# CycloneBoy/pdf_table

Measured on AMD Instinct MI355X. Metric: pages/s, higher is better.
Workload: dtype bf16

## Files before the change

include/pdftable_hip.h:

```cpp
#ifndef PDFTABLE_HIP_H
#define PDFTABLE_HIP_H

#include <stddef.h>
#include <stdint.h>

#ifdef __cplusplus
extern "C" {
#endif

#define PT_OK 0
#define PT_ERR_INVALID 1
#define PT_ERR_HIP 2
#define PT_ERR_STATE 3
#define PT_ERR_FORMAT 4

typedef struct pt_engine pt_engine;
typedef void* pt_stream;

int pt_engine_create(int device_id, pt_engine** out);
void pt_engine_destroy(pt_engine* e);
const char* pt_last_error(void);
int pt_abi_version(void);
int pt_engine_check(pt_engine* e);
int pt_engine_set_lstm_cluster(pt_engine* e, int on);
// ... 100 lines not shown
int pt_rec_forward_net(pt_engine* e, const uint16_t* d_gray, int n, int32_t* d_ids, float* d_maxlogit, pt_stream stream);
int pt_rec_preprocess(pt_engine* e, const uint8_t* d_pages_rgb, int n_pages, int h, int w, const pt_rec_line* d_lines,
                      const int64_t* h_crop_px, int n_lines, uint16_t* d_gray, pt_stream stream);

#define PT_CVIT_W 804
#define PT_CVIT_CHUNK_W 300
#define PT_CVIT_CHUNK_STEP 252
#define PT_CVIT_T 201
#define PT_CVIT_NCLS 7644
int pt_rec_cvit_forward(pt_engine* e, const uint8_t* d_pages_rgb, int n_pages, int h, int w, const pt_rec_line* d_lines,
                        const int64_t* h_crop_px, const int32_t* h_crop_wh, int n_lines, int32_t* d_ids, float* d_maxlogit,
                        pt_stream stream);
int pt_rec_cvit_forward_crops(pt_engine* e, const uint8_t* d_crops_rgb, const pt_rec_line* d_lines, const int64_t* h_crop_px,
                              const int32_t* h_crop_wh, int n_lines, int32_t* d_ids, float* d_maxlogit, pt_stream stream);
int pt_rec_cvit_forward_net(pt_engine* e, const float* d_gray, int layout, int n_lines, const int32_t* h_text_w, int32_t* d_ids,
                            float* d_maxlogit, pt_stream stream);
int pt_rec_cvit_preprocess_crops(pt_engine* e, const uint8_t* d_crops_rgb, const pt_rec_line* d_lines, const int64_t* h_crop_px,
                                 int n_lines, float* d_gray, pt_stream stream);

typedef struct pt_rec_pp_item {
  int32_t line;
  int32_t resized_w;
  int32_t img_w;
  int32_t reserved;
  int64_t out_off;
} pt_rec_pp_item;
int pt_rec_pp_preprocess(pt_engine* e, const uint8_t* d_pages_rgb, int n_pages, int h, int w, const pt_rec_line* d_lines,
                         const int64_t* h_crop_px, int n_lines, const pt_rec_pp_item* d_items, int n_items, int img_h,
                         int max_img_w, float* d_out, pt_stream stream);
int pt_rec_pp_preprocess_crops(pt_engine* e, const uint8_t* d_crops_rgb, const pt_rec_line* d_lines, const int64_t* h_crop_px,
                               int n_lines, const pt_rec_pp_item* d_items, int n_items, int img_h, int max_img_w, float* d_out,
                               pt_stream stream);

typedef struct pt_tsr_table {
  double minv[6];
  int32_t page, x0, y0, crop_w, crop_h, reserved;
} pt_tsr_table;

int pt_tsr_preprocess(pt_engine* e, const uint8_t* d_pages_rgb, int n_pages, int ph, int pw, const pt_tsr_table* d_tables,
                      int n, int inp_h, int inp_w, int bgr, uint16_t* d_out_bf16, pt_stream stream);

#define PT_TSR_CS_SMALL 8
#define PT_TSR_CS_FEAT 256
int pt_tsr_forward_net(pt_engine* e, const uint16_t* d_input_bf16, int n, int H, int W, float* d_hm, float* d_st,
                       float* d_wh, float* d_ax, float* d_cr, float* d_reg, pt_stream stream);

int pt_tsr_forward_net_wireless(pt_engine* e, const uint16_t* d_input_bf16, int n, int H, int W, float* d_hm, float* d_st,
                                float* d_wh, float* d_ax, float* d_cr, float* d_reg, pt_stream stream);

#define PT_TSR_MAX_CELLS 3000
int pt_tsr_decode(pt_engine* e, const float* d_hm, const float* d_st, const float* d_wh, const float* d_ax,
                  const float* d_cr, const float* d_reg, int n, int h, int w, int wiz_rev, float vis_thresh,
                  int32_t* d_counts, float* d_dets, float* d_logi, pt_stream stream);

int pt_tsr_forward_decode(pt_engine* e, const uint16_t* d_input_bf16, int n, int in_h, int in_w, int wiz_rev,
                          float vis_thresh, int32_t* d_counts, float* d_dets, float* d_logi, pt_stream stream);

int pt_centernet_forward_net(pt_engine* e, const uint16_t* d_input_bf16, int n, int H, int W, float* d_hm, float* d_v2c, float* d_c2v,
                             float* d_reg, pt_stream stream);

#define PT_CENTERNET_MAX_CELLS 1000
int pt_centernet_decode(pt_engine* e, const float* d_hm, const float* d_v2c, const float* d_c2v, const float* d_reg, int n, int h, int w,
                        const double* d_affine, int32_t* d_counts, float* d_cells, pt_stream stream);

int pt_tsr_process(pt_engine* e, const float* d_logi, const float* d_dets, const int32_t* h_counts, int n_tables,
                   int use_2dpe, float* d_logic, float* d_stacked, pt_stream stream);

int pt_op_conv2d(pt_engine* e, const uint16_t* d_in, int B, int H, int W, int Cin, const uint16_t* d_w_tiled,
                 const float* d_bias, int N, int ks, int stride, uint16_t* d_out, int out_cstride, int out_coff,
                 int rep, int shuffle_cout, const uint16_t* d_res, int res_mode, int relu, int split, int out_lo_off,
                 pt_stream stream);
int pt_op_conv1x1_ex(pt_engine* e, const uint16_t* d_in, int B, int H, int W, int Cin, const uint16_t* d_w_tiled, const float* d_bias,
                     int N, uint16_t* d_out, float* d_out_f32, int out_cstride, int n_valid, const float* d_res_f32, int relu,
                     const int32_t* d_ylimit, pt_stream stream);

int pt_op_dcn(pt_engine* e, const uint16_t* d_in, const float* d_om, int B, int H, int W, int C, const uint16_t* d_w_tiled,
              const float* d_bias, int N, uint16_t* d_out, int relu, int split, pt_stream stream);

int pt_op_dwconvt_up_add(pt_engine* e, const uint16_t* d_in, const float* d_w, const uint16_t* d_add, uint16_t* d_out, int B, int h, int w, int C,
                         int f, int split, pt_stream stream);
int pt_op_dcn_up_add(pt_engine* e, const uint16_t* d_in, const float* d_om, int B, int H, int W, int C, const uint16_t* d_w_tiled,
                     const float* d_bias, int N, uint16_t* d_out, int relu, int split, const uint16_t* d_up_in, int up_h, int up_w,
                     const float* d_up_w, int up_f, pt_stream stream);

int pt_op_stem7x7(pt_engine* e, const uint16_t* d_in, int B, int H, int W, const uint16_t* d_w, const float* d_bias,
                  uint16_t* d_out, int split, pt_stream stream);
int pt_op_maxpool3x3s2(pt_engine* e, const uint16_t* d_in, int B, int H, int W, int C, uint16_t* d_out, int split,
                       pt_stream stream);
int pt_op_db_head_final(pt_engine* e, const uint16_t* d_in, int B, int H, int W, const void* d_w, const float* d_bias,
                        float* d_prob, float* d_logits, int split, pt_stream stream);

int pt_op_dwconv(pt_engine* e, const uint16_t* d_in, int B, int H, int W, int C, const float* d_w_taps, const float* d_bias, int k,
                 int stride, int act, uint16_t* d_out, int split, pt_stream stream);
int pt_op_add(pt_engine* e, const uint16_t* d_a, const uint16_t* d_b, uint16_t* d_out, long long npix, int C, int split, pt_stream stream);
int pt_op_maxpool(pt_engine* e, const uint16_t* d_in, int B, int H, int W, int C, int k, int stride, int pad, uint16_t* d_out,
                  int split, pt_stream stream);
int pt_op_avgpool(pt_engine* e, const uint16_t* d_in, int B, int H, int W, int C, int k, uint16_t* d_out, int split, pt_stream stream);
int pt_op_chan_mean(pt_engine* e, const uint16_t* d_in, int B, int HW, int C, float* d_scratch, uint16_t* d_mean, int split, pt_stream stream);
int pt_op_chan_mean_scratch_floats(int B, int C);
int pt_op_scale_channels(pt_engine* e, const uint16_t* d_in, const uint16_t* d_gate, int B, int HW, int C, uint16_t* d_out,
                         int split, pt_stream stream);
int pt_op_act(pt_engine* e, const uint16_t* d_in, long long n_elems, int kind, float alpha, float beta, uint16_t* d_out, int C, int split,
              pt_stream stream);
int pt_op_copy_channels(pt_engine* e, const uint16_t* d_src, long long npix, int src_cstride, int src_coff, uint16_t* d_dst, int dst_cstride, int dst_coff,
                        int n, pt_stream stream);
int pt_op_upsample_nearest(pt_engine* e, const uint16_t* d_in, int B, int H, int W, int C, int factor, uint16_t* d_out, pt_stream stream);
int pt_op_mul(pt_engine* e, const uint16_t* d_a, const uint16_t* d_b, uint16_t* d_out, long long n_elems, int C, int split, pt_stream stream);
int pt_copy_bytes(pt_engine* e, const void* src, void* dst, long long nbytes, pt_stream stream);
int pt_op_layernorm(pt_engine* e, const uint16_t* d_in, long long rows, int c_pad, int c, const float* d_gamma, const float* d_beta, float eps,
                    uint16_t* d_out, int split, pt_stream stream);
int pt_op_softmax(pt_engine* e, const uint16_t* d_in, long long rows, int c_pad, int c, float* d_out_f32, uint16_t* d_out_bf16, int split, pt_stream stream);
int pt_op_attention(pt_engine* e, const uint16_t* d_qkv, int B, int T, int heads, int d, int qkv_cstride, float scale, uint16_t* d_out, int out_cstride,
                    int split, pt_stream stream);

int pt_op_cvit_mlp(pt_engine* e, const uint16_t* d_xb, long long rows, int C, const uint16_t* d_w1, const float* d_b1, const uint16_t* d_w2p,
                   const float* d_b2, float* d_x, pt_stream stream);
int pt_op_cvit_attention(pt_engine* e, const uint16_t* d_qkv, int nchunks, uint16_t* d_out, int split, pt_stream stream);
int pt_op_cvit_dwconv_ln(pt_engine* e, const float* d_x, int B, int H, int W, int C, const float* d_w49, const float* d_bias, const float* d_g,
                         const float* d_beta, uint16_t* d_out, int split, pt_stream stream);
int pt_op_cvit_ln(pt_engine* e, const float* d_x, long long rows, int C, const float* d_g, const float* d_beta, float eps, uint16_t* d_out, int split,
                  int mode, int H, int W, const int32_t* d_cmap, pt_stream stream);

int pt_op_lstm(pt_engine* e, const uint16_t* d_pregates, int pg_cstride, const uint16_t* d_r_packed, int T, int B, int H, int dirs, int reverse,
               uint16_t* d_y, int y_cstride, int split, pt_stream stream);
int pt_op_lstm_packed_elems(int H, int dirs, int split);

int pt_op_conv2d_rect(pt_engine* e, const uint16_t* d_in, int B, int H, int W, int Cin, const uint16_t* d_w_tiled, const float* d_bias, int N, int kh,
                      int kw, int sh, int sw, uint16_t* d_out, int out_cstride, int out_coff, int act, int split, int out_lo_off, pt_stream stream);
int pt_op_dwconv_rect(pt_engine* e, const uint16_t* d_in, int B, int H, int W, int C, const float* d_w_taps, const float* d_bias, int k, int sh, int sw,
                      int act, uint16_t* d_out, int split, pt_stream stream);
int pt_op_pool_rect(pt_engine* e, const uint16_t* d_in, int B, int H, int W, int C, int kind, int kh, int kw, uint16_t* d_out, int split,
                    pt_stream stream);

int pt_op_conv2d_large(pt_engine* e, const uint16_t* d_in, int B, int H, int W, int Cin, const uint16_t* d_w_tiled, const float* d_bias, int N, int kh,
                       int kw, uint16_t* d_out, int out_cstride, int out_coff, int act, int split, int out_lo_off, pt_stream stream);

int pt_op_affine_act(pt_engine* e, const uint16_t* d_in, long long npix, int Cpad, int C, const float* d_s1, const float* d_b1, const float* d_s2,
                     const float* d_b2, int act, uint16_t* d_out, int split, pt_stream stream);
int pt_op_db_tail(pt_engine* e, const uint16_t* d_in, int B, int H, int W, int Cpad, int C, int C1, const float* d_w1, const float* d_b1,
                  const float* d_w2, const float* d_b2, float* d_out, int split, pt_stream stream);

#define PT_CLS_SLOTS 4
#define PT_CLS_MAX_CLASSES 16
typedef struct pt_cls_image {
  int64_t offset;
  int32_t h, w;
} pt_cls_image;

int pt_cls_preprocess(pt_engine* e, const uint8_t* d_base, const pt_cls_image* d_images, int n, int max_h, int max_w,
                      int out_h, int out_w, uint16_t* d_out_bf16, pt_stream stream);
int pt_cls_forward_net(pt_engine* e, int slot, const uint16_t* d_input_bf16, int n, int in_h, int in_w, int textline,
                       float* d_logits, int* n_classes, pt_stream stream);
int pt_cls_forward(pt_engine* e, int slot, const uint8_t* d_base, const pt_cls_image* d_images, int n, int max_h, int max_w,
                   int out_h, int out_w, int textline, float* d_logits, int* n_classes, pt_stream stream);
int pt_cls_forward_lines(pt_engine* e, int slot, const uint8_t* d_pages_rgb, int n_pages, int h, int w,
                         const pt_rec_line* d_lines, const int64_t* h_crop_px, int n_lines, int max_crop_h, int max_crop_w,
                         int out_h, int out_w, int textline, float* d_logits, int* n_classes, pt_stream stream);
int pt_cls_forward_lines_direct(pt_engine* e, int slot, const uint8_t* d_pages_rgb, int n_pages, int h, int w,
                                const pt_rec_line* d_lines, int n_lines, int max_crop_h, int max_crop_w, int out_h, int out_w,
                                int textline, float* d_logits, int* n_classes, pt_stream stream);

#define PT_PROF_CONV3X3 0
#define PT_PROF_CONV1X1 1
#define PT_PROF_STEM 2
#define PT_PROF_OTHER 3
#define PT_PROF_NCLASS 4
// ... 33 lines not shown
```

pdf_table_amd/csrc/c_api.hip:

```cpp
#include <stdarg.h>
#include <stdio.h>
#include <stdlib.h>

#include <cmath>

#include "common.h"

namespace PT_FMT_NS {
namespace api {

static int ensure(void** buf, size_t* cap, size_t need);

int pt_engine_check(pt_engine* e) {
  PT_REQUIRE(e, "pt_engine_check: null engine");
  if (e->lstm_err && *e->lstm_err) {
    *e->lstm_err = 0;
    e->lstm_cluster = 0;
    pt_set_error("lstm_cluster_kernel: a workgroup waited > 2^22 polls for its peers -- the launch was not co-resident "
                 "(GPU shared with another process or stream?).  The recognition results since the last check are invalid; "
                 "this engine now uses the streaming LSTM kernel (pt_engine_set_lstm_cluster(e, 0)): run the batch again");
    return PT_ERR_HIP;
  }
  return PT_OK;
}
// ... 894 lines not shown
  bf16_t* xin = reinterpret_cast<bf16_t*>(e->cls_direct_in);
  for (int i0 = 0; i0 < n_lines; i0 += mb) {
    const int nb = (n_lines - i0) < mb ? (n_lines - i0) : mb;
    {
      PtProfScope ps(e, s, PT_PROF_OTHER, 0, "cls line resize+norm");
      rc = pt_launch_cls_line_resize_norm(d_pages_rgb, h, w, d_lines + i0, nb, max_crop_h, max_crop_w, out_h, out_w, e->cls_lut, x3, xin, s);
      if (rc != PT_OK) return rc;
    }
    rc = pt_pplcnet_forward_net(e, slot, xin, nb, out_h, out_w, textline, d_logits + (size_t)i0 * PT_CLS_MAX_CLASSES, n_classes, s,
                                PT_ARENA_CLS);
    if (rc != PT_OK) return rc;
  }
  return PT_OK;
}

int pt_op_conv2d(pt_engine* e, const uint16_t* d_in, int B, int H, int W, int Cin, const uint16_t* d_w_tiled,
                 const float* d_bias, int N, int ks, int stride, uint16_t* d_out, int out_cstride, int out_coff,
                 int rep, int shuffle_cout, const uint16_t* d_res, int res_mode, int relu, int split, int out_lo_off,
                 pt_stream stream) {
  PT_REQUIRE(e != nullptr, "pt_op_conv2d: null engine");
  ConvDesc d;
  d.in = d_in; d.B = B; d.H = H; d.W = W; d.Cin = Cin; d.w = d_w_tiled; d.bias = d_bias; d.N = N; d.ks = ks;
  d.stride = stride; d.out = d_out; d.out_cstride = out_cstride; d.out_coff = out_coff; d.rep = rep;
  d.shuffle_cout = shuffle_cout; d.res = d_res; d.res_mode = res_mode; d.relu = relu;
  d.split = split; d.out_lo_off = out_lo_off;
  return pt_launch_conv(e, d, reinterpret_cast<hipStream_t>(stream));
}

int pt_op_conv1x1_ex(pt_engine* e, const uint16_t* d_in, int B, int H, int W, int Cin, const uint16_t* d_w_tiled, const float* d_bias,
                     int N, uint16_t* d_out, float* d_out_f32, int out_cstride, int n_valid, const float* d_res_f32, int relu,
                     const int32_t* d_ylimit, pt_stream stream) {
  PT_REQUIRE(e != nullptr, "pt_op_conv1x1_ex: null engine");
  ConvDesc d;
  d.in = d_in; d.B = B; d.H = H; d.W = W; d.Cin = Cin; d.w = d_w_tiled; d.bias = d_bias; d.N = N; d.ks = 1; d.stride = 1;
  d.out = d_out_f32 ? nullptr : d_out; d.out_f32 = d_out_f32; d.out_cstride = out_cstride; d.n_valid = n_valid; d.res_f32 = d_res_f32;
  d.relu = relu; d.ylimit = d_ylimit;
  return pt_launch_conv(e, d, reinterpret_cast<hipStream_t>(stream));
}

int pt_op_stem7x7(pt_engine* e, const uint16_t* d_in, int B, int H, int W, const uint16_t* d_w, const float* d_bias,
                  uint16_t* d_out, int split, pt_stream stream) {
  PT_REQUIRE(e != nullptr, "pt_op_stem7x7: null engine");
  return pt_launch_stem7x7(e, d_in, B, H, W, d_w, d_bias, d_out, split, reinterpret_cast<hipStream_t>(stream));
}

int pt_op_maxpool3x3s2(pt_engine* e, const uint16_t* d_in, int B, int H, int W, int C, uint16_t* d_out, int split,
                       pt_stream stream) {
  PT_REQUIRE(e && d_in && d_out, "pt_op_maxpool3x3s2: bad arguments");
  return pt_launch_maxpool3x3s2(d_in, B, H, W, C, d_out, split, reinterpret_cast<hipStream_t>(stream));
}

int pt_op_db_head_final(pt_engine* e, const uint16_t* d_in, int B, int H, int W, const void* d_w, const float* d_bias,
                        float* d_prob, float* d_logits, int split, pt_stream stream) {
  PT_REQUIRE(e && d_in && d_w && d_bias && (d_prob || d_logits), "pt_op_db_head_final: bad arguments");
  return pt_launch_db_head_final(d_in, B, H, W, d_w, d_bias, d_prob, d_logits, split, reinterpret_cast<hipStream_t>(stream));
}

int pt_op_dcn(pt_engine* e, const uint16_t* d_in, const float* d_om, int B, int H, int W, int C, const uint16_t* d_w_tiled,
              const float* d_bias, int N, uint16_t* d_out, int relu, int split, pt_stream stream) {
  PT_REQUIRE(e && d_in && d_om && d_w_tiled && d_bias && d_out, "pt_op_dcn: null argument");
  PT_REQUIRE(B > 0 && H > 0 && W > 0, "pt_op_dcn: empty map (B=%d H=%d W=%d)", B, H, W);
  return pt_launch_dcn_fused(e, d_in, d_om, d_w_tiled, d_bias, d_out, B, H, W, C, N, split, relu, reinterpret_cast<hipStream_t>(stream));
}

int pt_op_dwconvt_up_add(pt_engine* e, const uint16_t* d_in, const float* d_w, const uint16_t* d_add, uint16_t* d_out, int B, int h, int w, int C,
                         int f, int split, pt_stream stream) {
  PT_REQUIRE(e && d_in && d_w && d_out, "pt_op_dwconvt_up_add: null argument");
  PT_REQUIRE(B > 0 && h > 0 && w > 0 && C > 0, "pt_op_dwconvt_up_add: empty map (B=%d h=%d w=%d C=%d)", B, h, w, C);
  return pt_launch_dwconvt_up_add(d_in, d_w, d_add, d_out, B, h, w, C, f, split, reinterpret_cast<hipStream_t>(stream));
}

int pt_op_dcn_up_add(pt_engine* e, const uint16_t* d_in, const float* d_om, int B, int H, int W, int C, const uint16_t* d_w_tiled,
                     const float* d_bias, int N, uint16_t* d_out, int relu, int split, const uint16_t* d_up_in, int up_h, int up_w,
                     const float* d_up_w, int up_f, pt_stream stream) {
  PT_REQUIRE(e && d_in && d_om && d_w_tiled && d_bias && d_out && d_up_in && d_up_w, "pt_op_dcn_up_add: null argument");
  PT_REQUIRE(B > 0 && H > 0 && W > 0, "pt_op_dcn_up_add: empty map (B=%d H=%d W=%d)", B, H, W);
  PT_REQUIRE(split == 0, "pt_op_dcn_up_add: the (hi | lo) modes keep the two launches (pt_op_dcn, pt_op_dwconvt_up_add)");
  PT_REQUIRE((up_f == 2 || up_f == 4) && up_h > 0 && up_w > 0 && up_h * up_f == H && up_w * up_f == W,
             "pt_op_dcn_up_add: a %dx%d map times %d is not the %dx%d output", up_h, up_w, up_f, H, W);
  return pt_launch_dcn_fused(e, d_in, d_om, d_w_tiled, d_bias, d_out, B, H, W, C, N, split, relu, reinterpret_cast<hipStream_t>(stream), nullptr, nullptr,
                             d_up_in, d_up_w, up_f);
}

int pt_profile_enable(pt_engine* e, int on) {
  PT_REQUIRE(e != nullptr, "pt_profile_enable: null engine");
  PT_REQUIRE(on >= 0 && on < 2 + PT_PROF_NCLASS, "pt_profile_enable: mode %d out of range", on);
  if (on && !e->prof.h_lims)
    PT_HIP_CHECK(hipHostMalloc(reinterpret_cast<void**>(&e->prof.h_lims), PtProfile::MAX_LIMS * sizeof(int), hipHostMallocDefault));
  e->prof.on = on;
  return PT_OK;
}

int pt_profile_read_labels(pt_engine* e, char* buf, int cap) {
  PT_REQUIRE(e && buf && cap > 0, "pt_profile_read_labels: bad arguments");
  PT_HIP_CHECK(hipDeviceSynchronize());
  struct Row { double ms = 0, flop = 0, bytes = 0; long long n = 0; };
  std::map<std::string, Row> rows;
  for (auto& p : e->prof.pending) {
    float ms = 0.f;
    if (hipEventElapsedTime(&ms, p.a, p.b) != hipSuccess) continue;
    double fl = p.flop;
    if (p.lim_slot >= 0 && p.rows > 0) {
      const int lim = e->prof.h_lims[p.lim_slot];
      fl *= (double)(lim < 0 ? 0 : (lim > p.rows ? p.rows : lim)) / p.rows;
    }
    Row& r = rows[p.label];
    r.ms += ms; r.flop += fl; r.bytes += p.bytes; r.n += 1;
  }
  std::string text;
  char line[160];
  for (auto& kv : rows) {
    snprintf(line, sizeof(line), "%s\t%lld\t%.6f\t%.6e\t%.6e\n", kv.first.c_str(), kv.second.n, kv.second.ms, kv.second.flop, kv.second.bytes);
    text += line;
  }
  PT_REQUIRE((int)text.size() + 1 <= cap, "pt_profile_read_labels: %d bytes needed, %d given", (int)text.size() + 1, cap);
  memcpy(buf, text.c_str(), text.size() + 1);
  for (auto& p : e->prof.pending) {
    (void)hipEventDestroy(p.a);
    (void)hipEventDestroy(p.b);
  }
  e->prof.pending.clear();
  e->prof.n_lims = 0;
  for (int i = 0; i < PT_PROF_NCLASS; ++i) { e->prof.ms[i] = 0; e->prof.launches[i] = 0; e->prof.flop[i] = 0; }
  return PT_OK;
}

int pt_profile_read(pt_engine* e, double* ms_per_class, long long* launches_per_class, double* flop_per_class) {
  PT_REQUIRE(e != nullptr, "pt_profile_read: null engine");
  PT_HIP_CHECK(hipDeviceSynchronize());
  const bool verbose = getenv("PT_PROF_VERBOSE") != nullptr;
  std::map<std::string, std::pair<double, int>> by_label;
  for (auto& p : e->prof.pending) {
    float ms = 0.f;
    if (hipEventElapsedTime(&ms, p.a, p.b) == hipSuccess) {
      if (verbose) { auto& r = by_label[p.label]; r.first += ms; r.second += 1; }
      e->prof.ms[p.cls] += ms;
      e->prof.launches[p.cls] += 1;
      double fl = p.flop;
      if (p.lim_slot >= 0 && p.rows > 0) {
        const int lim = e->prof.h_lims[p.lim_slot];
        fl *= (double)(lim < 0 ? 0 : (lim > p.rows ? p.rows : lim)) / p.rows;
      }
      e->prof.flop[p.cls] += fl;
    }
    (void)hipEventDestroy(p.a);
    (void)hipEventDestroy(p.b);
  }
  e->prof.pending.clear();
  e->prof.n_lims = 0;
  if (verbose)
    for (auto& kv : by_label)
      fprintf(stderr, "[pt_prof] %-40s n=%5d total=%9.3f ms avg=%8.4f ms\n", kv.first.c_str(), kv.second.second, kv.second.first,
              kv.second.first / kv.second.second);
  for (int i = 0; i < PT_PROF_NCLASS; ++i) {
    if (ms_per_class) ms_per_class[i] = e->prof.ms[i];
    if (launches_per_class) launches_per_class[i] = e->prof.launches[i];
    if (flop_per_class) flop_per_class[i] = e->prof.flop[i];
    e->prof.ms[i] = 0;
    e->prof.launches[i] = 0;
    e->prof.flop[i] = 0;
  }
  return PT_OK;
}

}
}
// ... 1 lines not shown
```

pdf_table_amd/csrc/common.h:

```cpp
#pragma once
#include <hip/hip_runtime.h>
#include <stdint.h>
#include <string.h>

#include <map>
#include <string>
#include <vector>

#include "../../include/pdftable_hip.h"
#include "act16.h"

typedef uint16_t bf16_t;

void pt_set_error(const char* fmt, ...);

#define PT_HIP_CHECK(expr)                                                                  \
  do {                                                                                      \
    hipError_t _e = (expr);                                                                 \
    if (_e != hipSuccess) {                                                                 \
      pt_set_error("%s failed: %s (%s:%d)", #expr, hipGetErrorString(_e), __FILE__, __LINE__); \
      return PT_ERR_HIP;                                                                    \
    }                                                                                       \
  } while (0)

// ... 138 lines not shown
  int lstm_max_cl = 0;
  int dcn_mfma = 0;
  int mtl_kv_fp8 = 0;
  int lstm_cluster = 1;
  void* rec_zero[2] = {nullptr, nullptr};
  bool rec_zero_valid[2] = {false, false};
  hipEvent_t rec_zero_ready[2] = {nullptr, nullptr};
  void* rec_limits = nullptr; size_t rec_limits_cap = 0;
  int rec_ragged = 1;
  std::vector<int> cvit_maps[16][2];
  int cvit_slot = 0;
  PtPinnedRing stage_ring;
  void* mtl_state = nullptr;
};

namespace PT_FMT_NS {

__device__ __forceinline__ void pt_warp_sample(const uint8_t* __restrict__ src, int ph, int pw, const double* m, int x, int y, int v[3]) {
  const double X0 = m[0] * x + m[1] * y + m[2];
  const double Y0 = m[3] * x + m[4] * y + m[5];
  double W = m[6] * x + m[7] * y + m[8];
  W = W != 0. ? 32. / W : 0.;
  const double fX = fmax(-2147483648., fmin(2147483647., X0 * W));
  const double fY = fmax(-2147483648., fmin(2147483647., Y0 * W));
  const long long Xi = (long long)rint(fX), Yi = (long long)rint(fY);
  const long long sx = Xi >> 5, sy = Yi >> 5;
  const int ax = (int)(Xi & 31), ay = (int)(Yi & 31);
  const int w00 = (32 - ay) * (32 - ax) * 32, w01 = (32 - ay) * ax * 32, w10 = ay * (32 - ax) * 32, w11 = ay * ax * 32;
  int acc[3] = {0, 0, 0};
  auto tap = [&](long long yy, long long xx, int wgt) {
    if (wgt && yy >= 0 && yy < ph && xx >= 0 && xx < pw) {
      const uint8_t* p = src + ((size_t)yy * pw + xx) * 3;
      acc[0] += p[0] * wgt; acc[1] += p[1] * wgt; acc[2] += p[2] * wgt;
    }
  };
  tap(sy, sx, w00); tap(sy, sx + 1, w01); tap(sy + 1, sx, w10); tap(sy + 1, sx + 1, w11);
#pragma unroll
  for (int c = 0; c < 3; ++c) {
    const int t = (acc[c] + (1 << 14)) >> 15;
    v[c] = t < 0 ? 0 : (t > 255 ? 255 : t);
  }
}

struct ConvDesc {
  const bf16_t* in = nullptr;
  int B = 0, H = 0, W = 0, Cin = 0;
  const bf16_t* in_more[3] = {nullptr, nullptr, nullptr};
  int seg_c[4] = {0, 0, 0, 0};
  int nseg = 1;
  const bf16_t* w = nullptr;
  const float* bias = nullptr;
  int N = 0;
  int ks = 3;
  int stride = 1;
  bf16_t* out = nullptr;
  int out_cstride = 0;
  int out_coff = 0;
  int rep = 1;
  int shuffle_cout = 0;
  const bf16_t* res = nullptr;
  int res_mode = 0;
  int relu = 0;
  const float* slope = nullptr;
  int pool = 0;
  const int* ylimit = nullptr;
  const int* xlimit = nullptr;
  const int* xlimit_cols = nullptr;
  const int* xlimit_rows = nullptr;
  const int* block_list = nullptr;
  int split = 0;
  int out_lo_off = 0;
  const void* head_w = nullptr;
  const float* head_b = nullptr;
  float* head_prob = nullptr;
  float* head_logits = nullptr;
  float* argmax_part = nullptr;
  int n_valid = 0;
  float* out_f32 = nullptr;
  const float* res_f32 = nullptr;
  unsigned tap_mask[8] = {0, 0, 0, 0, 0, 0, 0, 0};
  int xp_store = 0;
  int alg_n = 0;
  double alg_scale = 1.0;
};
int pt_launch_conv(pt_engine* e, const ConvDesc& d, hipStream_t s);
int pt_launch_crnn_conv01(pt_engine* e, const bf16_t* gray, int n, const float* w64x9, const float* b0, const bf16_t* w1, const float* b1, bf16_t* p1,
                          const int* xlimit, const int* xlimit_cols, hipStream_t s);
int pt_launch_dwpw(pt_engine* e, const bf16_t* in, int B, int H, int W, int C, const float* dw_w, const float* dw_b, int k, int stride, int dw_act,
                   const ConvDesc& pw, hipStream_t s);

int pt_launch_stem7x7(pt_engine* e, const bf16_t* in, int B, int H, int W, const bf16_t* w, const float* bias,
                      bf16_t* out, int split, hipStream_t s, int stride = 2, int n_valid = 0);

int pt_launch_det_preprocess(const uint8_t* pages, int n, int h, int w, int nh, int nw, int flavour, int split,
                             bf16_t* out, hipStream_t s);
int pt_launch_dcn_fused(pt_engine* e, const bf16_t* x, const float* om, const bf16_t* w, const float* bias, bf16_t* out,
                        int B, int H, int W, int C, int N, int split, int relu, hipStream_t s, const bf16_t* omw = nullptr, const float* omb = nullptr,
                        const bf16_t* up_in = nullptr, const float* up_w = nullptr, int up_f = 0);
bool pt_dcn_fuses_om(const pt_engine* e, int C, int split);
bool pt_dcn_fuses_up(const pt_engine* e, int C, int N, int split);
int pt_launch_dwconvt_up_add(const bf16_t* in, const float* w, const bf16_t* add, bf16_t* out, int B, int h, int wd, int C, int f, int split,
                             hipStream_t s);
int pt_launch_maxpool3x3s2(const bf16_t* in, int B, int H, int W, int C, bf16_t* out, int split, hipStream_t s);
int pt_launch_stem7x7_pool(pt_engine* e, const bf16_t* in, int B, int H, int W, const bf16_t* w, const float* bias, bf16_t* out,
                           hipStream_t s);
int pt_launch_db_head_final(const bf16_t* in, int B, int H, int W, const void* w4x64, const float* bias, float* prob,
                            float* logits, int split, hipStream_t s);
int pt_launch_db_head_mfma(const bf16_t* in, int B, int H, int W, const bf16_t* w3, const float* b3, const bf16_t* w6,
                           const float* b6, float* prob, float* logits, hipStream_t s, uint32_t* bitmap = nullptr, float thresh = 0.f);
int pt_launch_bitmap(const float* prob, int n, int H, int W, float thresh, int dilate, uint32_t* bitmap,
                     hipStream_t s);
int pt_launch_box_scores(const float* prob, int n, int H, int W, const float* boxes, int nb, float* scores,
                         hipStream_t s);

#define PT_SE_CHUNKS 64
int pt_launch_stem3x3s2(const bf16_t* in, const float* w, const float* b, bf16_t* out, int B, int H, int W, int split,
                        hipStream_t s, int variant);
int pt_launch_dwconv(const bf16_t* in, const float* w, const float* b, bf16_t* out, int B, int H, int W, int C, int k,
                     int stride, int act, int split, hipStream_t s, const float* slope);
int pt_launch_se(const bf16_t* x, const float* w1, const float* b1, const float* w2, const float* b2, float* gate,
                 bf16_t* out, int B, int HW, int C, int split, hipStream_t s, int hidden, int mode, float* part);
int pt_launch_add(const bf16_t* a, const bf16_t* b, bf16_t* out, long long npix, int C, int split, hipStream_t s);
int pt_launch_chan_mean(const bf16_t* x, int B, int HW, int C, int split, float* part, bf16_t* mean, int rows, hipStream_t s);
int pt_pplcnet_forward_net(pt_engine* e, int slot, const bf16_t* x, int n, int H, int W, int textline, float* logits,
                           int* n_classes, hipStream_t s, int arena);
int pt_launch_cls_resize_norm(const uint8_t* base, const pt_cls_image* images, int n, int max_h, int max_w, int OH, int OW,
                              const float* lut, int split, bf16_t* out, hipStream_t s);
int pt_launch_cls_desc_from_lines(const pt_rec_line* lines, const long long* off, int n, pt_cls_image* images, hipStream_t s);
int pt_launch_cls_line_resize_norm(const uint8_t* pages, int ph, int pw, const pt_rec_line* lines, int n, int max_h, int max_w, int OH,
                                   int OW, const float* lut, int split, bf16_t* out, hipStream_t s);
int pt_launch_dbnas_tail(const bf16_t* y, const float* tw, int B, int H4, int W4, int split, float* prob, float* logits,
                         hipStream_t s);
int pt_dbnas_forward_net(pt_engine* e, const bf16_t* x, int n, int H, int W, float* prob, float* logits, hipStream_t s);

int pt_launch_rec_offsets(const pt_rec_line* lines, int n, long long* off, hipStream_t s);
int pt_launch_rec_warp(const uint8_t* pages, int ph, int pw, const pt_rec_line* lines, int n_lines,
                       const long long* pix_off, uint8_t* crops, int max_crop_px, hipStream_t s);
int pt_launch_rec_resize_gray(const uint8_t* crops, const pt_rec_line* lines, const long long* pix_off, int n_lines,
                              int split, bf16_t* out, hipStream_t s);
int pt_launch_rec_pp_resize_norm(const uint8_t* crops, const pt_rec_line* lines, const long long* pix_off,
                                 const pt_rec_pp_item* items, int n_items, int img_h, int max_img_w, const float* lut, float* out,
                                 hipStream_t s);
struct PtCrnnLimits {
  int* lim[6];
  int* cols;
  int* glist;
  int* blist3a;
  int* blist2a;
  int* blist2b;
};
int pt_launch_rows_live_list(const int* lim, int n, int* glist, hipStream_t s);
int pt_launch_crnn_limits(const pt_rec_line* lines, int n, const PtCrnnLimits& L, hipStream_t s);
int pt_launch_crnn_fill(bf16_t* out, const bf16_t* ref, const int* lim, int tile_w, int div, int n, int rows, int W, int cs,
                        hipStream_t s, const int* end_lim = nullptr, int end_tile = 1);
int pt_launch_crnn_conv0_pool(const bf16_t* in, int n, int H, int W, const float* w64x9, const float* bias, int split,
                              bf16_t* out, hipStream_t s, const int* xlim = nullptr);
int pt_launch_maxpool_kxk(const bf16_t* in, int n, int H, int W, int C, int kh, int kw, int h2c, int split, bf16_t* out,
                          hipStream_t s);
int pt_launch_lstm(pt_engine* e, const bf16_t* gx, const bf16_t* whh, bf16_t* hout, int B, int T, int split, hipStream_t s);
int pt_launch_gemm_argmax(const bf16_t* A, long long M, int K, const bf16_t* W, const float* bias, int N, int* ids, float* maxv,
                          hipStream_t s);
int pt_launch_gemm_argmax_x3(const bf16_t* A, long long M, int K, const bf16_t* W3, const float* bias, int N, int n_real, int* ids, float* maxv,
                             void* scratch, hipStream_t s);
int pt_launch_gemm_rows_x3(const bf16_t* A, long long M, int K, const bf16_t* W3, const float* bias, int N, bf16_t* out, int relu, hipStream_t s,
                           const int* tlim = nullptr);
int pt_launch_gemm_rows(const bf16_t* A, long long M, int K, const bf16_t* W, const float* bias, int N, bf16_t* out, int relu,
                        hipStream_t s, const int* tlim = nullptr);
int pt_launch_argmax_reduce(const float* part, long long rows, int ntiles, int* ids, float* maxv, hipStream_t s);
int pt_crnn_forward_net(pt_engine* e, const bf16_t* gray, int n, int32_t* ids, float* maxlogit, hipStream_t s,
                        const pt_rec_line* d_lines = nullptr);

int pt_cvit_forward_net(pt_engine* e, const float* gray, int layout, int n, int32_t* ids, float* maxlogit, hipStream_t s,
                        const int* h_text_w = nullptr);
int pt_launch_rec_resize_gray_f32(const uint8_t* crops, const pt_rec_line* lines, const long long* pix_off, int n_lines, int tw,
                                  float* out, hipStream_t s);

int pt_mtl_backbone_forward_net(pt_engine* e, const bf16_t* x, int n, int H, int W, float* f3, hipStream_t s);
void pt_mtl_release(pt_engine* e);
int pt_mtl_preprocess(pt_engine* e, const uint8_t* pages, int ph, int pw, const pt_tsr_table* tabs, int n, int size, bf16_t* out, hipStream_t s);
int pt_mtl_decoder_config(pt_engine* e, int32_t* out13);
int pt_mtl_structure(pt_engine* e, const float* f3, int n, int hw, float* d_tag_logits, float* d_boxes, int32_t* h_lens, int32_t* h_cell_counts,
                     int force_redecode, hipStream_t s);
int pt_mtl_cells(pt_engine* e, int total, int32_t* d_cell_ids, float* d_cell_prob, float* d_cell_logits, int32_t* h_steps, int force_redecode,
                 hipStream_t s);

int pt_db_forward_net(pt_engine* e, const bf16_t* x, int n, int H, int W, float* prob, float* logits, hipStream_t s, uint32_t* bitmap = nullptr,
                      float thresh = 0.f, int* bitmap_done = nullptr);
int pt_launch_tsr_preprocess(const uint8_t* pages, int ph, int pw, const pt_tsr_table* tabs, int n, int H, int W, int bgr,
                             const float* lut, bf16_t* out, int split, hipStream_t s);
int pt_picodet_forward_net(pt_engine* e, const bf16_t* x, int n, int H, int W, float* h0, float* h1, float* h2, float* h3,
                          hipStream_t s);
int pt_launch_pico_candidates(const float* head, int B, int A, int ncls, int level, float thr_lo, int max_cands, float* cands,
                              int* counts, hipStream_t s);
int pt_lore_decode(pt_engine* e, const float* hm, const float* st, const float* wh, const float* ax, const float* cr,
                   const float* reg, int B, int H, int W, int wiz_rev, float vis_thresh, int* d_counts, float* d_dets,
                   float* d_logi, hipStream_t s);
void pt_lore_mosaic_rows(int B, int* rows_ax, int* rows_cr, int* rows_cell, int* rows_corner);
int pt_lore_decode_peaks(pt_engine* e, const float* hm, int B, int H, int W, int wiz_rev, float vis_thresh, int* d_counts,
                         const int** d_lim_cell, const int** d_lim_corner, hipStream_t s);
int pt_lore_peak_patches(pt_engine* e, const bf16_t* feat, int B, int H, int W, int C, int split, bf16_t* mos_cell,
                         bf16_t* mos_corner, hipStream_t s);
int pt_lore_decode_boxes(pt_engine* e, const float* reg_cell, const float* wh, const float* reg_corner, const float* st, int B,
                         int H, int W, const int** d_lim_ax, const int** d_lim_cr, hipStream_t s);
int pt_lore_patch_gather(pt_engine* e, const bf16_t* feat, int B, int H, int W, int C, int split, bf16_t* mos_ax, bf16_t* mos_cr,
                         hipStream_t s);
int pt_lore_decode_sparse(pt_engine* e, const float* ax_mos, const float* cr_mos, int B, int H, int W, float vis_thresh,
                          int* d_counts, float* d_dets, float* d_logi, hipStream_t s);
int pt_lore_forward_decode(pt_engine* e, const bf16_t* x, int n, int H, int W, int wiz_rev, float vis_thresh, int* d_counts,
                           float* d_dets, float* d_logi, hipStream_t s);
int pt_lore_wireless_forward_net(pt_engine* e, const bf16_t* x, int n, int H, int W, float* hm, float* st, float* wh,
                                 float* ax, float* cr, float* reg, hipStream_t s);
int pt_lore_process(pt_engine* e, const float* d_logi, const float* d_dets, const int32_t* h_counts, int n_tables,
                    int use_2dpe, float* d_logic, float* d_stacked, hipStream_t s);
int pt_lore_forward_net(pt_engine* e, const bf16_t* x, int n, int H, int W, float* hm, float* st, float* wh, float* ax,
                        float* cr, float* reg, hipStream_t s);
constexpr int PT_HEAT_CAP = 16384;
int pt_heat_peaks_topk(const float* hm, int B, int H, int W, float thr0, float thr1, int k0, int k1, float* sig, unsigned long long* keys,
                       int* cnt, unsigned long long* sorted, int* kept, hipStream_t s);
int pt_centernet_net(pt_engine* e, const bf16_t* x, int n, int H, int W, float* hm, float* v2c, float* c2v, float* reg, hipStream_t s);
int pt_centernet_decode_maps(pt_engine* e, const float* hm, const float* v2c, const float* c2v, const float* reg, int B, int H, int W,
                             const double* affine, int* d_counts, float* d_cells, hipStream_t s);

static inline int pt_split(const pt_engine* e) { return e->precision == PT_PRECISION_BF16X3 || e->precision == PT_PRECISION_F16X2; }
static inline int pt_f16x2(const pt_engine* e) { return e->precision == PT_PRECISION_F16X2; }

struct PtProfScope {
  pt_engine* e;
  hipStream_t s;
  int idx = -1;
  PtProfScope(pt_engine* e_, hipStream_t s_, int cls, double flop, const char* label = "") : e(e_), s(s_) {
    double bytes = 0;
    if (e) { bytes = e->prof.next_bytes; e->prof.next_bytes = 0; }
    if (e && e->prof.on && (e->prof.on == 1 || e->prof.on - 2 == cls)) {
      PtProfile::Pending p;
      p.bytes = bytes;
      if (hipEventCreate(&p.a) != hipSuccess || hipEventCreate(&p.b) != hipSuccess) return;
      p.cls = cls;
      p.flop = flop;
      strncpy(p.label, label, sizeof(p.label) - 1);
      p.label[sizeof(p.label) - 1] = 0;
      (void)hipEventRecord(p.a, s);
      e->prof.pending.push_back(p);
      idx = (int)e->prof.pending.size() - 1;
    }
  }
  ~PtProfScope() {
    if (idx >= 0) (void)hipEventRecord(e->prof.pending[idx].b, s);
  }
};

static inline int pt_model_format_ok(const PtModel& m, const char* what) {
  if (m.act_f16 != PT_ACT_F16) {
    pt_set_error("%s: the loaded weight blob holds %s tiles but the engine computes in %s (pack it with fmt=\"%s\" / set the matching precision)", what,
                 m.act_f16 ? "fp16" : "bf16", PT_FMT_NAME, PT_FMT_NAME);
    return 0;
  }
  return 1;
}

}
```

pdf_table_amd/csrc/conv_igemm.hip:

```cpp
#include <stdio.h>
#include <stdlib.h>

#include <type_traits>

#include "common.h"

namespace PT_FMT_NS {

typedef __attribute__((ext_vector_type(8))) __bf16 bf16x8;
typedef __attribute__((ext_vector_type(8))) _Float16 f16x8;
typedef __attribute__((ext_vector_type(16))) float f32x16;
typedef __attribute__((ext_vector_type(4))) float f32x4;
typedef __attribute__((ext_vector_type(4))) uint32_t u32x4;
typedef __attribute__((ext_vector_type(2))) uint32_t u32x2;

struct ConvK {
  const bf16_t* in;
  const bf16_t* w;
  const float* bias;
  bf16_t* out;
  const bf16_t* res;
  int B, H, W, Cin, Ho, Wo, N;
  int out_cstride, out_coff, rep, shuffle_cout, res_mode, relu;
  int tiles_x, tiles_y, n_tiles;
// ... 1230 lines not shown
        static_assert(C::SLOTS <= DPT * (NTAP - 1), "every DMA request has a tap");
      }
    });
    static_for<NTAP - 1>([&](auto tap_c) {
      constexpr int tap = decltype(tap_c)::value;
      constexpr int left = C::SLOTS - DPT * tap;
      constexpr int nd = MORE ? (left > DPT ? DPT : (left > 0 ? left : 0)) : 0;
      tap_groups<2 + C::MT, 2 * C::MT, nd>();
    });
    if constexpr (MORE) {
      asm volatile("s_waitcnt vmcnt(0)" ::: "memory");
      __syncthreads();
      load_frags(smem + (P ^ 1) * C::BUF_BYTES, 0, ((P + 1) * NTAP) & 1);
    }
    mma_tap((P * NTAP + NTAP - 1) & 1);
    tap_groups<MORE ? 2 + C::MT : 0, 2 * C::MT, 0>();
  };
  if constexpr (SKEW) {
    asm volatile("s_waitcnt vmcnt(0)" ::: "memory");
    __syncthreads();
    load_frags(smem, 0, 0);
    for (int c = 0; c + 2 < nslices; c += 2) {
      skew_slice(c, std::integral_constant<int, 0>{}, std::true_type{});
      skew_slice(c + 1, std::integral_constant<int, 1>{}, std::true_type{});
    }
    skew_slice(nslices - 2, std::integral_constant<int, 0>{}, std::true_type{});
    skew_slice(nslices - 1, std::integral_constant<int, 1>{}, std::false_type{});
  } else {
    static_assert(!PHASE, "phase convolutions: the SKEW loop only");
    for (int c = 0; c + 1 < nslices; ++c) slice_body(c, std::true_type{});
    slice_body(nslices - 1, std::false_type{});
  }

  if constexpr (DIRECT) {
    const int n0 = (NT == 1 ? nb : nb * 2 + wn) * 64;
    const DirectBias bs = direct_bias<2>(p, n0, qh);
    int bj = blk_b[0], xj = blk_x[0];
#pragma unroll
    for (int t = 1; t < C::NBLK; ++t)
      if ((C::MT * wm) / C::BR == t) { bj = blk_b[t]; xj = blk_x[t]; }
    if (xj >= p.Wo) return;
#pragma unroll
    for (int m = 0; m < C::MT; ++m) epilogue_direct_row<2>(p, acc[m], bs, bj, oy0 + (C::MT * wm) % C::BR + m, xj, lx, n0, qh, nullptr);
    return;
  }
  float* stage = reinterpret_cast<float*>(smem);
#pragma unroll
  for (int pass = 0; pass < 2; ++pass) {
    __syncthreads();
    const bool mine = NT == 1 ? ((wave / (NWV / 2)) == pass) : (wn == pass);
    if (mine) {
      const int rbase = NT == 1 ? C::MT * (wave % (NWV / 2)) : C::MT * wm;
#pragma unroll
      for (int m = 0; m < C::MT; ++m)
#pragma unroll
        for (int n = 0; n < 2; ++n)
#pragma unroll
          for (int r = 0; r < 16; ++r) {
            const int tx = (r & 3) + 8 * (r >> 2) + 4 * qh;
            stage[((rbase + m) * 32 + tx) * 64 + n * 32 + lx] = acc[m][n][r];
          }
    }
    __syncthreads();
    if constexpr (C::NBLK > 1) {
      static_assert(NT == 2 || C::NBLK == 1, "blocked tiles: one pass = all rows of one 64-channel half");
#pragma unroll 1
      for (int j = 0; j < C::NBLK; ++j) {
        int bj = blk_b[0], xj = blk_x[0];
#pragma unroll
        for (int t = 1; t < C::NBLK; ++t)
          if (j == t) { bj = blk_b[t]; xj = blk_x[t]; }
        if (xj < p.Wo) epilogue_store<C::BR, 32, C::NTHR, 2>(p, stage + j * C::BR * 32 * 64, tid, bj, 0, xj, (nb * 2 + pass) * 64);
      }
    } else if (NT == 1) {
      epilogue_store<C::PASS_ROWS, 32, C::NTHR, 0>(p, stage, tid, b, oy0 + C::PASS_ROWS * pass, ox0, nb * 64);
    } else {
      epilogue_store<C::PASS_ROWS, 32, C::NTHR, 0>(p, stage, tid, b, oy0, ox0, (nb * 2 + pass) * 64);
    }
  }
#endif
}

template <int NT, int NWV, int S>
__global__ __launch_bounds__(64 * NWV, 2) void conv3x3_pipe_persist_kernel(ConvK p) {
#if defined(__HIP_DEVICE_COMPILE__)
  a16_kernel_enter();
  using C = PipeCfg<NT, NWV, 0, S>;
  static_assert(C::NBLK == 1, "ordinary tiles");
  extern __shared__ __attribute__((aligned(16))) char smem[];
  const int tid = threadIdx.x;
  const int lane = tid & 63;
  const int wave = __builtin_amdgcn_readfirstlane(tid >> 6);
  const int lx = lane & 31, qh = lane >> 5;
  const int wm = NT == 1 ? wave : (wave >> 1);
  const int wn = NT == 1 ? 0 : (wave & 1);
  const int G = gridDim.x;
  const int Lw = xcd_remap(blockIdx.x, G);
  const int t0 = (int)((long long)Lw * p.total_tiles / G), t1 = (int)((long long)(Lw + 1) * p.total_tiles / G);
  if (t0 >= t1) return;
  const int in_cs = p.Cin;
  const int nch32 = p.Cin >> 5, nslices = nch32 * 2;

  constexpr int OOB = 0x7FFFF000;
  int meta[C::SLOTS];
  bool is_in[C::SLOTS];
  int dst[C::SLOTS];
#pragma unroll
  for (int j = 0; j < C::SLOTS; ++j) {
    int k = wave + NWV * j;
    if (k >= C::T_INSTR) k = C::T_INSTR - 1;
    is_in[j] = k < C::IN_INSTR;
    dst[j] = k * 1024;
    if (is_in[j]) {
      const int U = k * 64 + lane;
      const int pix = U >> 1;
      const int pr = pix / C::TWIN, sx = pix - pr * C::TWIN;
      const int q = (U & 1) ^ ((sx >> 3) & 1);
      const int ix = S == 1 ? sx : (sx < C::XEVEN ? 2 * sx : 2 * (sx - C::XEVEN) + 1);
      meta[j] = U < C::IN_UNITS ? (pr | (ix << 8) | (q << 16)) : -1;
    } else {
      const int U = (k - C::IN_INSTR) * 64 + lane;
      const int row = U >> 1;
      const int tap = row / C::NW, n = row - tap * C::NW;
      const int hq = (U & 1) ^ ((row >> 3) & 1);
      meta[j] = (int)((((size_t)(n >> 6) * nch32 * (9 * 64 * 32)) + (tap * 64 + (n & 63)) * 32 + hq * 8) * 2);
    }
  }
  struct Tile { int b, oy0, ox0, nb; };
  auto decode = [&](int L) {
    Tile t;
    t.nb = L % p.n_tiles;
    L /= p.n_tiles;
    const int txi = L % p.tiles_x;
    L /= p.tiles_x;
    const int tyi = L % p.tiles_y;
    t.b = L / p.tiles_y;
    t.ox0 = txi * C::TW;
    t.oy0 = tyi * C::TH;
    return t;
  };
  auto offsets = [&](const Tile& t, int (&vo)[C::SLOTS]) {
#pragma unroll
    for (int j = 0; j < C::SLOTS; ++j) {
      if (is_in[j]) {
        const int m = meta[j];
        const int gy = t.oy0 * S - 1 + (m & 0xFF), gx = t.ox0 * S - 1 + ((m >> 8) & 0xFF);
        const bool inside = m >= 0 && (unsigned)gy < (unsigned)p.H && (unsigned)gx < (unsigned)p.W;
        vo[j] = inside ? ((gy * p.W + gx) * in_cs + ((m >> 16) & 1) * 8) * 2 : OOB;
      } else {
        vo[j] = meta[j];
      }
    }
  };
  auto rsrc_in = [&](const Tile& t) { return __builtin_amdgcn_make_buffer_rsrc(const_cast<bf16_t*>(p.in + (size_t)t.b * p.H * p.W * in_cs), 0, OOB, 0x00020000); };
  auto rsrc_w = [&](const Tile& t) { return __builtin_amdgcn_make_buffer_rsrc(const_cast<bf16_t*>(p.w + (size_t)(NT * t.nb) * nch32 * (9 * 64 * 32)), 0, OOB, 0x00020000); };
  auto in_off = [&](int slice) { return slice << 4; };
  auto w_off = [&](int slice) { return (slice >> 1) * (9 * 64 * 32) + (slice & 1) * 16; };

  f32x16 acc[C::MT][2];
#pragma unroll
  for (int m = 0; m < C::MT; ++m)
#pragma unroll
    for (int n = 0; n < 2; ++n)
#pragma unroll
      for (int r = 0; r < 16; ++r) acc[m][n][r] = 0.f;
  int a_lane[3];
#pragma unroll
  for (int s = 0; s < 3; ++s) {
    const int soff = S == 1 ? s : ((s & 1) * C::XEVEN + (s >> 1));
    a_lane[s] = ((C::MT * wm * S) * C::TWIN + lx + soff) * 32 + ((qh ^ (((lx + soff) >> 3) & 1)) << 4);
  }
  const int b_lane = C::IN_BYTES + (wn * 64 + lx) * 32 + ((qh ^ ((lx >> 3) & 1)) << 4);
  bf16x8 fa[2][C::MT], fb[2][2];
  auto load_frags = [&](const char* sb, int tap, int slot) {
    const int r = tap / 3, s = tap - 3 * r;
    fb[slot][0] = *reinterpret_cast<const bf16x8*>(sb + b_lane + (tap * C::NW) * 32);
    fb[slot][1] = *reinterpret_cast<const bf16x8*>(sb + b_lane + (tap * C::NW + 32) * 32);
#pragma unroll
    for (int m = 0; m < C::MT; ++m) fa[slot][m] = *reinterpret_cast<const bf16x8*>(sb + a_lane[s] + ((S * m + r) * C::TWIN) * 32);
  };
  auto mma_tap = [&](int slot) {
#pragma unroll
    for (int m = 0; m < C::MT; ++m) {
      acc[m][0] = mfma_32x32x16_a16(fb[slot][0], fa[slot][m], acc[m][0]);
      acc[m][1] = mfma_32x32x16_a16(fb[slot][1], fa[slot][m], acc[m][1]);
    }
  };

  Tile cur = decode(t0);
  int vo[C::SLOTS];
  offsets(cur, vo);
  __amdgpu_buffer_rsrc_t r_in = rsrc_in(cur), r_w = rsrc_w(cur);
#pragma unroll
  for (int j = 0; j < C::SLOTS; ++j)
    __builtin_amdgcn_raw_ptr_buffer_load_lds(is_in[j] ? r_in : r_w, (__attribute__((address_space(3))) void*)(smem + dst[j]), 16, vo[j], 0, 0, 0);
  asm volatile("s_waitcnt vmcnt(0)" ::: "memory");
  __syncthreads();
  load_frags(smem, 0, 0);

  for (int ti = t0; ti < t1; ++ti) {
    auto skew_slice = [&](int c, auto par_tag, auto last_tag, int oi, int ow) {
      constexpr int P = decltype(par_tag)::value;
      constexpr bool LAST = decltype(last_tag)::value;
      constexpr int NTAP = 9;
      constexpr int DPT = (C::SLOTS + NTAP - 2) / (NTAP - 1) > 2 ? (C::SLOTS + NTAP - 2) / (NTAP - 1) : 2;
      const char* sb = smem + P * C::BUF_BYTES;
      static_for<NTAP - 1>([&](auto tap_c) {
        constexpr int tap = decltype(tap_c)::value;
        load_frags(sb, tap + 1, (P * NTAP + tap + 1) & 1);
        mma_tap((P * NTAP + tap) & 1);
#pragma unroll
        for (int j = DPT * tap; j < DPT * tap + DPT && j < C::SLOTS; ++j)
          __builtin_amdgcn_raw_ptr_buffer_load_lds(is_in[j] ? r_in : r_w, (__attribute__((address_space(3))) void*)(smem + (P ^ 1) * C::BUF_BYTES + dst[j]), 16, vo[j],
                                                   (is_in[j] ? oi : ow) * 2, 0, 0);
        static_assert(C::SLOTS <= DPT * (NTAP - 1), "every DMA request has a tap");
      });
      static_for<NTAP - 1>([&](auto tap_c) {
        constexpr int tap = decltype(tap_c)::value;
        constexpr int left = C::SLOTS - DPT * tap;
        constexpr int nd = left > DPT ? DPT : (left > 0 ? left : 0);
        tap_groups<2 + C::MT, 2 * C::MT, nd>();
      });
      asm volatile("s_waitcnt vmcnt(0)" ::: "memory");
      __syncthreads();
      if constexpr (!LAST) load_frags(smem + (P ^ 1) * C::BUF_BYTES, 0, ((P + 1) * NTAP) & 1);
      mma_tap((P * NTAP + NTAP - 1) & 1);
      tap_groups<LAST ? 0 : 2 + C::MT, 2 * C::MT, 0>();
    };
    for (int c = 0; c + 2 < nslices; c += 2) {
      skew_slice(c, std::integral_constant<int, 0>{}, std::false_type{}, in_off(c + 1), w_off(c + 1));
      skew_slice(c + 1, std::integral_constant<int, 1>{}, std::false_type{}, in_off(c + 2), w_off(c + 2));
    }
    skew_slice(nslices - 2, std::integral_constant<int, 0>{}, std::false_type{}, in_off(nslices - 1), w_off(nslices - 1));
    const Tile done = cur;
    {
      const bool has_next = ti + 1 < t1;
      cur = decode(has_next ? ti + 1 : ti);
      offsets(cur, vo);
      if (!has_next) {
#pragma unroll
        for (int j = 0; j < C::SLOTS; ++j) vo[j] = OOB;
      }
      r_in = rsrc_in(cur);
      r_w = rsrc_w(cur);
    }
    skew_slice(nslices - 1, std::integral_constant<int, 1>{}, std::true_type{}, 0, 0);
    {
      const int n0 = (NT == 1 ? done.nb : done.nb * 2 + wn) * 64;
      const DirectBias bs = direct_bias<2>(p, n0, qh);
#pragma unroll
      for (int m = 0; m < C::MT; ++m) {
        epilogue_direct_row<2>(p, acc[m], bs, done.b, done.oy0 + C::MT * wm + m, done.ox0, lx, n0, qh, nullptr);
#pragma unroll
        for (int n = 0; n < 2; ++n)
#pragma unroll
          for (int r = 0; r < 16; ++r) acc[m][n][r] = 0.f;
      }
    }
    load_frags(smem, 0, 0);
  }
#endif
}

struct GemmPipeCfg {
  static constexpr int NWV = 8, NTHR = 512, MT = 4, NG = 16;
  static constexpr int KS = 64, NW = 128;
  static constexpr int A_BYTES = NG * 32 * KS * 2, W_BYTES = NW * KS * 2, BUF_BYTES = A_BYTES + W_BYTES;
  static constexpr int A_INSTR = A_BYTES / 1024, W_INSTR = W_BYTES / 1024, SLOTS = (A_INSTR + W_INSTR) / NWV;
  static constexpr int SMEM = 2 * BUF_BYTES;
  static_assert(A_INSTR % NWV == 0 && W_INSTR % NWV == 0, "a slot is an A or a W request for every wave alike");
};

template <bool LIST>
__global__ __launch_bounds__(512, 2) void gemm_pipe_kernel(ConvK p) {
#if defined(__HIP_DEVICE_COMPILE__)
  a16_kernel_enter();
  using C = GemmPipeCfg;
  extern __shared__ __attribute__((aligned(16))) char smem[];
  const int tid = threadIdx.x;
  const int lane = tid & 63;
  const int wave = __builtin_amdgcn_readfirstlane(tid >> 6);
  const int lx = lane & 31, qh = lane >> 5;
  const int wm = wave >> 1, wn = wave & 1;

  const int L = LIST ? (int)blockIdx.x : xcd_remap(blockIdx.x, gridDim.x);
  const int nb = L % p.n_tiles, ti = L / p.n_tiles;
  const long long M = (long long)p.B * p.H * p.W;
  const int n_groups = (int)(M >> 5);
  int cnt = n_groups;
  if (LIST) {
    cnt = p.blist[0];
    if (ti * C::NG >= cnt) return;
  }
  auto group_of = [&](int j) {
    const int i = ti * C::NG + j;
    if (i >= cnt) return -1;
    return LIST ? p.blist[1 + i] : i;
  };
  const int K = p.Cin, nslices = K >> 6;
  const bf16_t* wt = p.w + (size_t)(2 * nb) * (K >> 5) * 2048;
  constexpr int OOB = 0x7FFFF000;
  const int g0 = group_of(0);
  const __amdgpu_buffer_rsrc_t r_a = __builtin_amdgcn_make_buffer_rsrc(const_cast<bf16_t*>(p.in + (size_t)g0 * 32 * K), 0, OOB, 0x00020000);
  const __amdgpu_buffer_rsrc_t r_w = __builtin_amdgcn_make_buffer_rsrc(const_cast<bf16_t*>(wt), 0, OOB, 0x00020000);
  int voff[C::SLOTS];
#pragma unroll
  for (int j = 0; j < C::SLOTS; ++j) {
    const int k = wave + C::NWV * j;
    if (j < C::A_INSTR / C::NWV) {
      const int U = k * 64 + lane, r = U >> 3, c = (U & 7) ^ ((r >> 1) & 7);
      const int g = group_of(r >> 5);
      const long long off = ((long long)(g - g0) * 32 + (r & 31)) * K + c * 8;
      voff[j] = (g >= 0 && off * 2 < OOB) ? (int)(off * 2) : OOB;
    } else {
      const int U = (k - C::A_INSTR) * 64 + lane, n = U >> 3, c = (U & 7) ^ ((n >> 1) & 7);
      voff[j] = (int)((((size_t)(n >> 6) * (K >> 5) + (c >> 2)) * 2048 + (n & 63) * 32 + (c & 3) * 8) * 2);
    }
  }
  auto issue_one = [&](int j, int slice, int buf) {
    const bool is_a = j < C::A_INSTR / C::NWV;
    __builtin_amdgcn_raw_ptr_buffer_load_lds(is_a ? r_a : r_w, (__attribute__((address_space(3))) void*)(smem + buf * C::BUF_BYTES + (wave + C::NWV * j) * 1024), 16,
                                             voff[j], is_a ? slice * 128 : slice * 2 * 2048 * 2, 0, 0);
  };

  f32x16 acc[C::MT][2];
#pragma unroll
  for (int m = 0; m < C::MT; ++m)
#pragma unroll
    for (int n = 0; n < 2; ++n)
#pragma unroll
      for (int r = 0; r < 16; ++r) acc[m][n][r] = 0.f;

  int a_lane[4], b_lane[4];
#pragma unroll
  for (int kk = 0; kk < 4; ++kk) {
    const int slot = ((kk * 2 + qh) ^ ((lx >> 1) & 7)) << 4;
    a_lane[kk] = (C::MT * wm) * 4096 + lx * 128 + slot;
    b_lane[kk] = C::A_BYTES + (wn * 64 + lx) * 128 + slot;
  }
  bf16x8 fa[2][C::MT], fb[2][2];
  auto load_frags = [&](const char* sb, int kk, int slot) {
    fb[slot][0] = *reinterpret_cast<const bf16x8*>(sb + b_lane[kk]);
    fb[slot][1] = *reinterpret_cast<const bf16x8*>(sb + b_lane[kk] + 4096);
// ... 1316 lines not shown
  PT_REQUIRE(nblk > 0 && nblk < (1ll << 31), "conv grid out of range (%lld blocks)", nblk);
  char label[48];
  snprintf(label, sizeof(label), "conv3x3 %s%s %d->%d @%dx%d%s", S == 2 ? "s2 v3" : "v3", NWV == 4 ? "h" : "", k.Cin, k.N, k.Ho, k.Wo, k.split ? " x3" : "");
  PtProfScope prof(e, s, PT_PROF_CONV3X3, flop, label);
  hipLaunchKernelGGL((conv3x3_dma16_kernel<NT, NWV, S>), dim3((unsigned)nblk), dim3(C::NTHR), C::SMEM, s, k,
                     reinterpret_cast<const bf16_t*>(e->zero_page));
  PT_HIP_CHECK(hipGetLastError());
  return PT_OK;
}

template <int NT, int NWV, bool SKEW, int BR = 0, bool DIRECT = false, int S = 1, bool PHASE = false>
static int launch_pipe(pt_engine* e, ConvK& k, hipStream_t s, double flop) {
  using C = PipeCfg<NT, NWV, BR, S>;
  static bool attr_done = false;
  if (!attr_done) {
    PT_HIP_CHECK(hipFuncSetAttribute(reinterpret_cast<const void*>(&conv3x3_pipe_kernel<NT, NWV, SKEW, BR, DIRECT, S, PHASE>), hipFuncAttributeMaxDynamicSharedMemorySize, C::SMEM));
    attr_done = true;
  }
  k.n_tiles = k.N / C::NW;
  long long nblk;
  if (C::NBLK == 1) {
    k.tiles_x = (k.Wo + C::TW - 1) / C::TW;
    k.tiles_y = (k.Ho + C::TH - 1) / C::TH;
    nblk = (long long)k.B * k.tiles_x * k.tiles_y * k.n_tiles;
  } else if (k.blist) {
    k.tiles_x = (int)(((long long)k.B * (k.Wo / 32) + C::NBLK - 1) / C::NBLK);
    k.tiles_y = 1;
    nblk = (long long)k.tiles_x * k.n_tiles;
  } else {
    k.tiles_x = (k.Wo + C::NBLK * 32 - 1) / (C::NBLK * 32);
    k.tiles_y = 1;
    nblk = (long long)k.B * k.tiles_x * k.n_tiles;
  }
  PT_REQUIRE(nblk > 0 && nblk < (1ll << 31), "conv grid out of range (%lld blocks)", nblk);
  char label[48];
  if (C::NBLK == 1) snprintf(label, sizeof(label), "conv3x3 %sv4%s%s %d->%d @%dx%d%s", S == 2 ? "s2 " : "", NWV == 4 ? "h" : "", PHASE ? "p" : "", k.Cin, k.N, k.Ho, k.Wo, k.split ? " x3" : "");
  else snprintf(label, sizeof(label), "conv3x3 v4b %d->%d @%dx%d%s", k.Cin, k.N, k.Ho, k.Wo, k.split ? " x3" : "");
  int lim_slot = -1;
  {
    PtProfScope prof(e, s, PT_PROF_CONV3X3, flop, label);
    hipLaunchKernelGGL((conv3x3_pipe_kernel<NT, NWV, SKEW, BR, DIRECT, S, PHASE>), dim3((unsigned)nblk), dim3(C::NTHR), C::SMEM, s, k, reinterpret_cast<const bf16_t*>(e->zero_page));
    if (k.xcols && prof.idx >= 0 && e->prof.h_lims && e->prof.n_lims < PtProfile::MAX_LIMS) {
      auto& pd = e->prof.pending[prof.idx];
      pd.lim_slot = lim_slot = e->prof.n_lims++;
      pd.rows = k.B * k.Wo;
    }
  }
  if (lim_slot >= 0) (void)hipMemcpyAsync(e->prof.h_lims + lim_slot, k.xcols, sizeof(int), hipMemcpyDeviceToHost, s);
  PT_HIP_CHECK(hipGetLastError());
  return PT_OK;
}

template <int NT, int NWV, int S>
static int launch_pipe_persist(pt_engine* e, ConvK& k, hipStream_t s, double flop) {
  using C = PipeCfg<NT, NWV, 0, S>;
  static bool attr_done = false;
  if (!attr_done) {
    PT_HIP_CHECK(hipFuncSetAttribute(reinterpret_cast<const void*>(&conv3x3_pipe_persist_kernel<NT, NWV, S>), hipFuncAttributeMaxDynamicSharedMemorySize, 2 * C::BUF_BYTES));
    attr_done = true;
  }
  k.n_tiles = k.N / C::NW;
  k.tiles_x = (k.Wo + C::TW - 1) / C::TW;
  k.tiles_y = (k.Ho + C::TH - 1) / C::TH;
  const long long total = (long long)k.B * k.tiles_x * k.tiles_y * k.n_tiles;
  PT_REQUIRE(total > 0 && total < (1ll << 31), "conv grid out of range (%lld tiles)", total);
  k.total_tiles = (int)total;
  const int per_cu = 2 * C::BUF_BYTES <= 80 * 1024 ? 2 : 1;
  long long grid = (long long)e->num_cu * per_cu;
  if (const char* gv = getenv("PT_CONV_PERSIST_GRID")) {
    const int gg = atoi(gv);
    if (gg > 0) grid = gg;
  }
  if (grid > total) grid = total;
  char label[48];
  snprintf(label, sizeof(label), "conv3x3 %sv5%s %d->%d @%dx%d", S == 2 ? "s2 " : "", NWV == 4 ? "h" : "", k.Cin, k.N, k.Ho, k.Wo);
  {
    PtProfScope prof(e, s, PT_PROF_CONV3X3, flop, label);
    hipLaunchKernelGGL((conv3x3_pipe_persist_kernel<NT, NWV, S>), dim3((unsigned)grid), dim3(C::NTHR), 2 * C::BUF_BYTES, s, k);
  }
  PT_HIP_CHECK(hipGetLastError());
  return PT_OK;
}

static int launch_gemm_pipe(pt_engine* e, ConvK& k, hipStream_t s, double flop) {
  using C = GemmPipeCfg;
  static bool attr_done = false;
  if (!attr_done) {
    PT_HIP_CHECK(hipFuncSetAttribute(reinterpret_cast<const void*>(&gemm_pipe_kernel<false>), hipFuncAttributeMaxDynamicSharedMemorySize, C::SMEM));
    PT_HIP_CHECK(hipFuncSetAttribute(reinterpret_cast<const void*>(&gemm_pipe_kernel<true>), hipFuncAttributeMaxDynamicSharedMemorySize, C::SMEM));
    attr_done = true;
  }
  const long long M = (long long)k.B * k.H * k.W, groups = M / 32;
  {
    const char* xv = getenv("PT_GEMM_XP");
    k.xp_store = !(xv && xv[0] == '0') && !k.out_f32;
  }
  k.n_tiles = k.N / C::NW;
  k.tiles_x = (int)((groups + C::NG - 1) / C::NG);
  k.tiles_y = 1;
  const long long nblk = (long long)k.tiles_x * k.n_tiles;
  PT_REQUIRE(nblk > 0 && nblk < (1ll << 31), "gemm grid out of range (%lld blocks)", nblk);
  char label[48];
  if (k.argmax_part) snprintf(label, sizeof(label), "classifier gemm+argmax");
  else snprintf(label, sizeof(label), "gemm %d->%d @%dx%d", k.Cin, k.N, k.Ho, k.Wo);
  int lim_slot = -1;
  {
    PtProfScope prof(e, s, PT_PROF_CONV1X1, flop, label);
    if (k.blist) hipLaunchKernelGGL((gemm_pipe_kernel<true>), dim3((unsigned)nblk), dim3(C::NTHR), C::SMEM, s, k);
    else hipLaunchKernelGGL((gemm_pipe_kernel<false>), dim3((unsigned)nblk), dim3(C::NTHR), C::SMEM, s, k);
    if (k.xcols && prof.idx >= 0 && e->prof.h_lims && e->prof.n_lims < PtProfile::MAX_LIMS) {
      auto& pd = e->prof.pending[prof.idx];
      pd.lim_slot = lim_slot = e->prof.n_lims++;
      pd.rows = k.xlimit_rows ? k.Ho * k.Wo : k.B * k.Wo;
    }
  }
  if (lim_slot >= 0) (void)hipMemcpyAsync(e->prof.h_lims + lim_slot, k.xcols, sizeof(int), hipMemcpyDeviceToHost, s);
  PT_HIP_CHECK(hipGetLastError());
  return PT_OK;
}

static int launch_ws64(pt_engine* e, ConvK& k, hipStream_t s, double flop) {
  using C = Ws64Cfg;
  static bool attr_done = false;
  if (!attr_done) {
    PT_HIP_CHECK(hipFuncSetAttribute(reinterpret_cast<const void*>(&conv3x3_ws64_kernel), hipFuncAttributeMaxDynamicSharedMemorySize, C::SMEM));
    attr_done = true;
  }
  if (!e->zero_page) {
    PT_HIP_CHECK(hipMalloc(&e->zero_page, 8192));
    PT_HIP_CHECK(hipMemset(e->zero_page, 0, 8192));
  }
  k.tiles_x = (k.Wo + C::TW - 1) / C::TW;
  k.tiles_y = (k.Ho + C::TH - 1) / C::TH;
  k.n_tiles = 1;
  const long long total = (long long)k.B * k.tiles_x * k.tiles_y;
  PT_REQUIRE(total > 0 && total < (1ll << 30), "conv grid out of range (%lld tiles)", total);
  k.total_tiles = (int)total;
  unsigned nblk = (unsigned)(total < e->num_cu ? total : e->num_cu);
  if (const char* gv = getenv("PT_CONV_WS64_GRID")) {
    const int g = atoi(gv);
    if (g > 0 && (unsigned)g < nblk) nblk = (unsigned)g;
  }
  char label[48];
  snprintf(label, sizeof(label), "conv3x3 ws %d->%d @%dx%d", k.Cin, k.N, k.Ho, k.Wo);
  PtProfScope prof(e, s, PT_PROF_CONV3X3, flop, label);
  hipLaunchKernelGGL(conv3x3_ws64_kernel, dim3(nblk), dim3(C::NTHR), C::SMEM, s, k, reinterpret_cast<const bf16_t*>(e->zero_page));
  PT_HIP_CHECK(hipGetLastError());
  return PT_OK;
}

static int conv_variant() {
  static int v = -1;
  if (v < 0) {
    const char* s = getenv("PT_CONV_VARIANT");
    v = s ? atoi(s) : 3;
  }
  return v;
}

int pt_launch_conv(pt_engine* e, const ConvDesc& d, hipStream_t s) {
  PT_REQUIRE(d.in && d.w && d.bias && (d.out || d.out_f32 || d.head_w || d.argmax_part), "conv: null pointer");
  PT_REQUIRE(d.Cin % 32 == 0 && d.Cin > 0, "conv: Cin=%d must be a positive multiple of 32", d.Cin);
  PT_REQUIRE(d.N % 64 == 0 && d.N > 0, "conv: N=%d must be a positive multiple of 64", d.N);
  PT_REQUIRE((d.ks == 1 || d.ks == 3) && (d.stride == 1 || d.stride == 2), "conv: ks=%d stride=%d unsupported", d.ks,
             d.stride);
  PT_REQUIRE(!(d.shuffle_cout && (d.rep != 1 || d.shuffle_cout % 64 != 0 || d.N != 4 * d.shuffle_cout)),
             "conv: bad pixel-shuffle configuration");
  PT_REQUIRE(d.rep >= 1 && d.out_cstride % 8 == 0 && d.out_coff % 8 == 0, "conv: bad output layout");
  ConvK k;
  memset(&k, 0, sizeof(k));
  k.n_valid = d.n_valid; k.out_f32 = d.out_f32; k.res_f32 = d.res_f32;
  PT_REQUIRE(!d.res_f32 || d.out_f32, "conv: fp32 residual needs the fp32 output path");
  PT_REQUIRE(d.n_valid % 8 == 0 && d.n_valid <= d.N, "conv: n_valid=%d must be a multiple of 8 and <= N", d.n_valid);
  PT_REQUIRE(!(d.out_f32 && (d.rep != 1 || d.shuffle_cout)), "conv: fp32 output only on the plain store path");
  k.in = d.in; k.w = d.w; k.bias = d.bias; k.out = d.out; k.res = d.res;
  k.nseg = d.nseg;
  if (d.nseg > 1) {
    PT_REQUIRE(d.nseg <= 4 && d.ks == 1 && d.stride == 1, "conv: K over several tensors needs a 1x1 stride-1 layer and <= 4 segments");
    int sum = 0;
    for (int i = 0; i < d.nseg; ++i) {
      PT_REQUIRE(d.seg_c[i] > 0 && d.seg_c[i] % 32 == 0 && (i == 0 || d.in_more[i - 1]), "conv: bad K segment %d", i);
      sum += d.seg_c[i];
    }
    PT_REQUIRE(sum == d.Cin, "conv: K segments sum to %d channels, Cin is %d", sum, d.Cin);
    k.in1 = d.in_more[0]; k.in2 = d.in_more[1]; k.in3 = d.in_more[2];
    k.segc0 = d.seg_c[0]; k.segc1 = d.seg_c[1]; k.segc2 = d.seg_c[2]; k.segc3 = d.seg_c[3];
  }
  k.B = d.B; k.H = d.H; k.W = d.W; k.Cin = d.Cin; k.N = d.N;
  const int pad = d.ks / 2;
  k.Ho = (d.H + 2 * pad - d.ks) / d.stride + 1;
  k.Wo = (d.W + 2 * pad - d.ks) / d.stride + 1;
  k.out_cstride = d.out_cstride; k.out_coff = d.out_coff; k.rep = d.rep; k.shuffle_cout = d.shuffle_cout;
  k.res_mode = d.res ? d.res_mode : 0; k.relu = d.relu; k.slope = d.slope; k.ylimit = d.ylimit; k.pool = d.pool;
  k.xlimit = d.xlimit; k.xlimit_rows = d.xlimit_rows; k.xcols = (d.xlimit || d.xlimit_rows) ? d.xlimit_cols : nullptr;
  {
    const char* bl = getenv("PT_CONV_BLOCK_LIST");
    k.blist = (d.xlimit && d.block_list && d.ks == 3 && d.stride == 1 && k.Ho <= 4 && k.Wo > 32 && k.Wo % 32 == 0 && !(bl && bl[0] == '0')) ? d.block_list : nullptr;
  }
  PT_REQUIRE(!d.xlimit_rows || (d.ks == 1 && d.stride == 1 && !d.ylimit && !d.xlimit), "conv: row-wise column limits need a 1x1 stride-1 layer");
  PT_REQUIRE(!d.xlimit || (d.ks == 3 && d.stride == 1 && !d.ylimit), "conv: column limits need a 3x3 stride-1 layer");
  PT_REQUIRE(!d.pool || (d.ks == 3 && d.stride == 1 && !d.res && !d.shuffle_cout && d.rep == 1 && !d.out_f32 && !d.argmax_part && !d.head_w && !d.n_valid && d.relu <= 1 && k.Ho % 2 == 0 && (d.pool != 1 || k.Wo % 2 == 0)),
             "conv: fused pooling needs a plain 3x3 stride-1 layer with even output size");
  PT_REQUIRE(d.relu != 3 || d.slope, "conv: PReLU needs the slope tensor");
  k.split = d.split; k.out_lo_off = d.out_lo_off;
  for (int i = 0; i < 8; ++i) k.tap_mask[i] = d.tap_mask[i];
  {
    const char* xv = getenv("PT_CONV_XP");
    k.xp_store = (xv ? atoi(xv) : d.xp_store) && !d.out_f32;
  }
  k.head_w = d.head_w; k.head_b = d.head_b; k.head_prob = d.head_prob; k.head_logits = d.head_logits;
  k.argmax_part = d.argmax_part;
  if (d.head_w) PT_REQUIRE(d.shuffle_cout == 64 && d.head_b && (d.head_prob || d.head_logits), "conv: bad fused-head configuration");
  if (k.res_mode == 2) PT_REQUIRE(k.Ho % 2 == 0 && k.Wo % 2 == 0, "conv: half-res residual needs even output size");
  const int n_alg = d.alg_n ? d.alg_n : (d.n_valid ? d.n_valid : d.N);
  const double flop = 2.0 * k.B * k.Ho * k.Wo * (double)n_alg * d.Cin * d.ks * d.ks * d.alg_scale;
  {
    const double mact = d.split ? 2.0 : 1.0, osz = d.out_f32 ? 4.0 : 2.0 * mact;
    const double in_px = (d.ks == 1 && d.stride == 2) ? (double)k.B * k.Ho * k.Wo : (double)d.B * d.H * d.W;
    const double nstore = d.shuffle_cout ? d.N : (d.n_valid ? d.n_valid : d.N);
    double by = in_px * d.Cin * 2.0 * mact + (double)k.B * k.Ho * k.Wo * d.rep * d.rep * nstore * osz * d.alg_scale;
    if (d.res || d.res_f32) by += (double)k.B * k.Ho * k.Wo * nstore * (d.res_f32 ? 4.0 : 2.0 * mact) / (d.res_mode == 2 ? 4.0 : 1.0);
    by += (double)d.N * d.Cin * d.ks * d.ks * 2.0 * (d.split == 2 ? 2 : (d.split ? 3 : 1));
    e->prof.next_bytes = by;
  }
  if (d.ks == 3 && d.stride == 2 && !d.split && d.N % 128 == 0 && d.Cin % 32 == 0 && d.Cin >= 64 && k.Ho >= 8 && !d.head_w && !d.argmax_part && !d.n_valid &&
      !d.out_f32 && !d.res_f32 && !d.res && d.relu < 2 && !d.ylimit && !d.xlimit && !d.xlimit_rows && !d.pool && d.rep == 1 && !d.shuffle_cout && use_dma_kernel()) {
    static int s2 = -1;
    if (s2 < 0) { const char* ev = getenv("PT_CONV_S2_DMA"); s2 = ev ? atoi(ev) : 1; }
    bool masked = false;
    for (int i = 0; i < 8; ++i) masked = masked || d.tap_mask[i] != 0;
    const char* pv2 = getenv("PT_CONV_PIPE");
    if (s2 && !masked && !(pv2 && pv2[0] == '0')) return launch_pipe<2, 8, true, 0, true, 2>(e, k, s, flop);
    if (s2 && !masked) return launch_dma16<2, 8, 2>(e, k, s, flop);
  }
  if (d.ks == 3 && d.stride == 1 && !d.head_w && !d.argmax_part && !d.n_valid && !d.out_f32 && !d.res_f32 && d.relu < 2 && !d.ylimit && !d.xlimit && !d.pool && d.split != 2 && use_dma_kernel()) {
    const int cv = conv_variant();
    const char* ws_ev = getenv("PT_CONV_WS64");
    const int ws64 = ws_ev ? atoi(ws_ev) : 1;
    bool masked = false;
    for (int i = 0; i < 8; ++i) masked = masked || d.tap_mask[i] != 0;
    if (ws64 && cv == 3 && !d.split && d.Cin == 64 && d.N == 64 && d.rep == 1 && !d.shuffle_cout && d.res_mode <= 1 && !masked &&
        (ws64 == 2 || (long long)k.B * ((k.Ho + 15) / 16) * ((k.Wo + 31) / 32) >= 4ll * e->num_cu))
      return launch_ws64(e, k, s, flop);
    const bool v3ok = (d.N % 128 == 0) ? k.Ho >= 12 : k.Ho >= 24;
    const bool wide = d.Cin >= 128;
    int pick = 0;
    if (cv == 3 && v3ok) pick = 3;
    else if (cv == 1 && wide && k.Ho >= 120) pick = 3;
    static int half = -2;
    if (half == -2) { const char* ev = getenv("PT_CONV_HALF"); half = ev ? atoi(ev) : -1; }
    bool use_half = half == 1;
    if (half < 0 && pick == 3) {
      const bool nt2 = d.N % 128 == 0;
      const long long full = (long long)k.B * ((k.Ho + (nt2 ? 15 : 31)) / (nt2 ? 16 : 32)) * ((k.Wo + 31) / 32) * (d.N / (nt2 ? 128 : 64));
      use_half = d.Cin <= 128 || (full < 2ll * e->num_cu && full % e->num_cu != 0);
    }
    const char* pv = getenv("PT_CONV_PIPE");
    bool phase = masked && d.N == 256;
    for (int i = 0; i < 8 && phase; ++i) {
      unsigned mk = 0;
      if (i < 4)
        for (int r = i >> 1; r < (i >> 1) + 2; ++r)
          for (int q = i & 1; q < (i & 1) + 2; ++q) mk |= 1u << (r * 3 + q);
      phase = d.tap_mask[i] == mk;
    }
    if (phase && cv == 3 && v3ok && !(pv && atoi(pv) < 3)) return launch_pipe<2, 8, true, 0, false, 1, true>(e, k, s, flop);
    const int pipe = masked ? 0 : (pv ? atoi(pv) : 4);
    if (pick == 3 && pipe == 1) {
      if (use_half) return launch_pipe<1, 4, false>(e, k, s, flop);
      return d.N % 128 == 0 ? launch_pipe<2, 8, false>(e, k, s, flop) : launch_pipe<1, 8, false>(e, k, s, flop);
    }
    if (pick == 3 && pipe >= 2) {
      const bool direct = pipe >= 3 && !k.split && !k.pool && !k.shuffle_cout;
      const bool nt2 = d.N % 128 == 0;
      const long long tiles = (long long)k.B * ((k.Ho + (nt2 ? 15 : 31)) / (nt2 ? 16 : 32)) * ((k.Wo + 31) / 32) * (d.N / (nt2 ? 128 : 64));
      if (use_half && half < 0 && direct && pipe >= 4 && d.Cin == 64 && nt2 && !d.res && tiles >= 2ll * e->num_cu) use_half = false;
      if (direct && pipe >= 4 && (!use_half || pipe >= 5) && !k.xlimit && !k.xlimit_rows && !k.blist) {
        if (tiles >= 2ll * e->num_cu || pipe >= 5)
          return nt2 ? launch_pipe_persist<2, 8, 1>(e, k, s, flop) : launch_pipe_persist<1, 8, 1>(e, k, s, flop);
      }
      if (direct) {
        if (use_half) return launch_pipe<1, 4, true, 0, true>(e, k, s, flop);
        return d.N % 128 == 0 ? launch_pipe<2, 8, true, 0, true>(e, k, s, flop) : launch_pipe<1, 8, true, 0, true>(e, k, s, flop);
      }
      if (use_half) return launch_pipe<1, 4, true>(e, k, s, flop);
      return d.N % 128 == 0 ? launch_pipe<2, 8, true>(e, k, s, flop) : launch_pipe<1, 8, true>(e, k, s, flop);
    }
    if (pick == 3 && use_half) return launch_dma16<1, 4>(e, k, s, flop);
    if (pick == 3) return d.N % 128 == 0 ? launch_dma16<2, 8>(e, k, s, flop) : launch_dma16<1, 8>(e, k, s, flop);
  }
  if (d.ks == 3 && d.stride == 1 && (k.Ho == 4 || k.Ho == 8) && k.H == k.Ho && k.Wo % 32 == 0 && k.Wo > 32 && d.N % 128 == 0 && d.Cin >= 128 && !d.head_w &&
      !d.argmax_part && !d.n_valid && !d.out_f32 && !d.res_f32 && !d.res && d.relu < 2 && !d.ylimit && !d.xlimit_rows && d.rep == 1 && !d.shuffle_cout &&
      d.split != 2 && use_dma_kernel()) {
    const char* pb = getenv("PT_CONV_PIPE_BLOCKS");
    const char* pv = getenv("PT_CONV_PIPE");
    bool masked = false;
    for (int i = 0; i < 8; ++i) masked = masked || d.tap_mask[i] != 0;
    if (!masked && !(pb && pb[0] == '0') && !(pv && pv[0] == '0')) {
      if (d.xlimit && d.block_list) k.blist = d.block_list;
      if (!k.split && !k.pool && !(pv && atoi(pv) < 3))
        return k.Ho == 4 ? launch_pipe<2, 8, true, 4, true>(e, k, s, flop) : launch_pipe<2, 8, true, 8, true>(e, k, s, flop);
      return k.Ho == 4 ? launch_pipe<2, 8, true, 4>(e, k, s, flop) : launch_pipe<2, 8, true, 8>(e, k, s, flop);
    }
  }
  if (d.ks == 3 && d.stride == 1 && k.Ho <= 4 && k.Wo > 32) return launch_cfg<3, 1, 1>(e, k, s, flop);
  if (d.ks == 3 && d.stride == 1) return launch_cfg<3, 1>(e, k, s, flop);
// ... 186 lines not shown
```

pdf_table_amd/csrc/lore_decode.hip:

```cpp
#include "common.h"

namespace PT_FMT_NS {

namespace {

constexpr int CAP = PT_HEAT_CAP;
constexpr int K_CELLS = 3000, K_CORNERS = 5000;

__global__ __launch_bounds__(256) void lore_sigmoid_kernel(const float* __restrict__ hm, float* __restrict__ sig,
                                                            long long npix) {
  a16_kernel_enter();
  const long long i = (long long)blockIdx.x * blockDim.x + threadIdx.x;
  if (i >= npix) return;
  sig[2 * i] = 1.f / (1.f + expf(-hm[8 * i]));
  sig[2 * i + 1] = 1.f / (1.f + expf(-hm[8 * i + 1]));
}

__device__ __forceinline__ bool heat_is_peak(const float* __restrict__ sb, int H, int W, int y, int x, int cls, float thr, float& s) {
  s = sb[((size_t)y * W + x) * 2 + cls];
  if (!(s >= thr)) return false;
  for (int dy = -1; dy <= 1; ++dy)
    for (int dx = -1; dx <= 1; ++dx) {
      const int yy = y + dy, xx = x + dx;
      if (yy < 0 || yy >= H || xx < 0 || xx >= W) continue;
      if (sb[((size_t)yy * W + xx) * 2 + cls] > s) return false;
    }
  return true;
}

__device__ __forceinline__ unsigned long long heat_key(float s, unsigned pixel) {
  return ((unsigned long long)__float_as_uint(s) << 32) | (unsigned long long)(0xFFFFFFFFu - pixel);
}

template <int NTHR>
__global__ __launch_bounds__(NTHR) void lore_peaks_kernel(const float* __restrict__ sig, int B, int H, int W, float thr_cell,
                                                          float thr_corner, unsigned long long* __restrict__ keys,
                                                          int* __restrict__ counts) {
  a16_kernel_enter();
  const long long i = (long long)blockIdx.x * blockDim.x + threadIdx.x;
  const bool live = i < (long long)B * H * W;
  const long long ic = live ? i : 0;
  const int x = (int)(ic % W), y = (int)((ic / W) % H), b = (int)(ic / ((long long)W * H));
  const float* sb = sig + (size_t)b * H * W * 2;
  const bool uniform = ((long long)H * W) % NTHR == 0;
  __shared__ int s_cnt[2][NTHR / 64];
  __shared__ int s_base[2];
  const int wave = threadIdx.x >> 6;
  for (int cls = 0; cls < 2; ++cls) {
    const float s = sb[((size_t)y * W + x) * 2 + cls];
    bool peak = live && (s >= (cls ? thr_corner : thr_cell));
    if (peak) {
      for (int dy = -1; dy <= 1 && peak; ++dy)
        for (int dx = -1; dx <= 1; ++dx) {
          const int yy = y + dy, xx = x + dx;
          if (yy < 0 || yy >= H || xx < 0 || xx >= W) continue;
          if (sb[((size_t)yy * W + xx) * 2 + cls] > s) { peak = false; break; }
        }
    }
    const int list = b * 2 + cls;
    int slot = -1;
    if (uniform) {
      const unsigned long long m = __ballot(peak);
      if ((threadIdx.x & 63) == 0) s_cnt[cls][wave] = __popcll(m);
      __syncthreads();
      if (threadIdx.x == 0) {
        int tot = 0;
        for (int k = 0; k < NTHR / 64; ++k) tot += s_cnt[cls][k];
        s_base[cls] = tot ? atomicAdd(&counts[list], tot) : 0;
      }
      __syncthreads();
      if (peak) {
        int base = s_base[cls];
        for (int k = 0; k < wave; ++k) base += s_cnt[cls][k];
        slot = base + __popcll(m & ((1ull << (threadIdx.x & 63)) - 1ull));
      }
    } else if (peak) {
      slot = atomicAdd(&counts[list], 1);
    }
    if (peak && slot < CAP)
      keys[(size_t)list * CAP + slot] = ((unsigned long long)__float_as_uint(s) << 32) |
                                        (unsigned long long)(0xFFFFFFFFu - (unsigned)(y * W + x));
  }
}

__device__ int heat_count_from(const float* __restrict__ sb, int H, int W, int cls, float thr, unsigned long long lo, int* s_acc) {
  const int npix = H * W;
  if (threadIdx.x == 0) *s_acc = 0;
  __syncthreads();
  int c = 0;
  for (int i = threadIdx.x; i < npix; i += blockDim.x) {
    float s;
    if (heat_is_peak(sb, H, W, i / W, i % W, cls, thr, s) && heat_key(s, (unsigned)i) >= lo) ++c;
  }
#pragma unroll
  for (int d = 32; d > 0; d >>= 1) c += __shfl_xor(c, d);
  if ((threadIdx.x & 63) == 0 && c) atomicAdd(s_acc, c);
  __syncthreads();
  const int tot = *s_acc;
// ... 261 lines not shown
  if (p >= ncell) return;
  const int r = order ? (int)(0xFFFFFFFFu - (unsigned)(order[(size_t)b * stride + p] & 0xFFFFFFFFull)) : p;
  const float* cellbox = boxes + ((size_t)(2 * b) * stride) * 12;
  const float* here = rev ? rev + ((size_t)b * stride + p) * 12 : cellbox + (size_t)p * 12;
  __shared__ int pos[5];
  if (threadIdx.x < 5) {
    const int m = (int)threadIdx.x - 1;
    long long cc;
    if (m < 0) {
      cc = __float_as_int(cellbox[(size_t)r * 12 + 11]);
    } else {
      const float f = here[2 * m] + (float)W * rintf(here[2 * m + 1]);
      cc = (long long)rintf(f);
      if (!(cc < (long long)H * W)) cc = 0;
      if (cc < 0) cc = 0;
    }
    pos[threadIdx.x] = (int)cc;
  }
  __syncthreads();
  const int cs = split ? 2 * C : C, ppx = cs / 8;
  const long long j = sp_base[b] + p;
  for (int i = threadIdx.x; i < 5 * 9 * ppx; i += 256) {
    const int piece = i % ppx, tap = (i / ppx) % 9, k = i / (9 * ppx);
    const int y = pos[k] / W + tap / 3 - 1, x = pos[k] % W + tap % 3 - 1;
    uint4 v = make_uint4(0u, 0u, 0u, 0u);
    if ((unsigned)y < (unsigned)H && (unsigned)x < (unsigned)W)
      v = *reinterpret_cast<const uint4*>(feat + (((size_t)b * H + y) * W + x) * cs + piece * 8);
    const long long pj = k == 0 ? j : 4 * j + (k - 1);
    bf16_t* dst = (k == 0 ? mos_ax : mos_cr) + (size_t)pj * 9 * cs + patch_off(tap, piece * 8, C);
    *reinterpret_cast<uint4*>(dst) = v;
  }
}

__global__ __launch_bounds__(256) void lore_gather_kernel(const float* __restrict__ rev, const float* __restrict__ boxes,
                                                           const unsigned long long* __restrict__ order,
                                                           const int* __restrict__ counts, int stride, int H, int W,
                                                           const float* __restrict__ ax, const float* __restrict__ cr,
                                                           float vis_thresh, float* __restrict__ dets,
                                                           float* __restrict__ logi, int* __restrict__ n_valid,
                                                           const int* __restrict__ sp_base) {
  a16_kernel_enter();
  const int b = blockIdx.y, p = blockIdx.x, c = threadIdx.x;
  const int ncell = counts[2 * b];
  if (p >= ncell) return;
  const int r = order ? (int)(0xFFFFFFFFu - (unsigned)(order[(size_t)b * stride + p] & 0xFFFFFFFFull)) : p;
  const float* cellbox = boxes + ((size_t)(2 * b) * stride) * 12;
  const float* src = rev ? rev + ((size_t)b * stride + r) * 12 : cellbox + (size_t)r * 12;
  const float* here = rev ? rev + ((size_t)b * stride + p) * 12 : cellbox + (size_t)p * 12;
  const float score = src[8];
  if (c < 8) dets[((size_t)b * K_CELLS + p) * 9 + c] = src[c];
  if (c == 8) {
    dets[((size_t)b * K_CELLS + p) * 9 + 8] = score;
    if (score >= vis_thresh) atomicAdd(&n_valid[b], 1);
  }
  if (sp_base) {
    const long long j = sp_base[b] + p;
    float v = ax[mosaic_centre(j) * 256 + c];
    float crs = 0.f;
#pragma unroll
    for (int m = 0; m < 4; ++m) crs += cr[mosaic_centre(4 * j + m) * 256 + c];
    logi[((size_t)b * K_CELLS + p) * 256 + c] = v + crs;
    return;
  }
  const int centre = __float_as_int(cellbox[(size_t)r * 12 + 11]);
  const size_t fb = (size_t)b * H * W;
  float v = ax[(fb + centre) * 256 + c];
  float crs = 0.f;
  const long long npix = (long long)H * W;
#pragma unroll
  for (int m = 0; m < 4; ++m) {
    const float f = here[2 * m] + (float)W * rintf(here[2 * m + 1]);
    long long cc = (long long)rintf(f);
    if (!(cc < npix)) cc = 0;
    if (cc < 0) cc = 0;
    crs += cr[(fb + cc) * 256 + c];
  }
  logi[((size_t)b * K_CELLS + p) * 256 + c] = v + crs;
}

}

int pt_heat_peaks_topk(const float* hm, int B, int H, int W, float thr0, float thr1, int k0, int k1, float* sig, unsigned long long* keys,
                       int* cnt, unsigned long long* sorted, int* kept, hipStream_t s) {
  PT_REQUIRE(hm && sig && keys && cnt && sorted && kept && B > 0 && k0 <= CAP && k1 <= CAP, "heat peaks: bad arguments");
  PT_REQUIRE((long long)H * W < (1ll << 31), "heat peaks: map too large");
  static bool attr_done = false;
  if (!attr_done) {
    PT_HIP_CHECK(hipFuncSetAttribute(reinterpret_cast<const void*>(&lore_sort_kernel),
                                     hipFuncAttributeMaxDynamicSharedMemorySize, CAP * 8));
    attr_done = true;
  }
  const size_t npix = (size_t)B * H * W;
  hipLaunchKernelGGL(lore_sigmoid_kernel, dim3((unsigned)((npix + 255) / 256)), dim3(256), 0, s, hm, sig, (long long)npix);
  hipLaunchKernelGGL(lore_peaks_kernel<1024>, dim3((unsigned)((npix + 1023) / 1024)), dim3(1024), 0, s, sig, B, H, W, thr0, thr1, keys, cnt);
  hipLaunchKernelGGL(lore_sort_kernel, dim3(2 * B), dim3(1024), CAP * 8, s, keys, cnt, 1, CAP, k0, k1, sorted, CAP, kept,
                     (const float*)sig, H, W, thr0, thr1);
  PT_HIP_CHECK(hipGetLastError());
  return PT_OK;
}

struct DecodeState {
  int* cnt;
  unsigned long long *sorted, *keys2, *sorted2;
  float *boxes, *rev;
  int *sp_base, *sp_lim;
  int *pk_base, *pk_lim;
  int wiz_rev;
};

static int decode_peaks(pt_engine* e, const float* hm, int B, int H, int W, int wiz_rev, float vis_thresh, int* d_counts,
                        DecodeState* ds, hipStream_t s) {
  PT_REQUIRE((long long)H * W < (1ll << 31), "tsr decode: map too large");
  const size_t npix = (size_t)B * H * W;
  size_t off = 0;
  auto carve = [&](size_t bytes) { size_t o = off; off = (off + bytes + 255) & ~size_t(255); return o; };
  const size_t o_sig = carve(npix * 2 * 4), o_cnt = carve((size_t)B * 5 * 4), o_keys = carve((size_t)2 * B * CAP * 8),
               o_sorted = carve((size_t)2 * B * CAP * 8), o_boxes = carve((size_t)2 * B * CAP * 12 * 4),
               o_rev = carve((size_t)B * CAP * 12 * 4), o_keys2 = carve((size_t)B * CAP * 8),
               o_sorted2 = carve((size_t)B * CAP * 8), o_sp = carve((size_t)(3 * B + 4) * 4);
  if (off > e->tsr_scratch_cap) {
    PT_HIP_CHECK(hipDeviceSynchronize());
    if (e->tsr_scratch) PT_HIP_CHECK(hipFree(e->tsr_scratch));
    e->tsr_scratch = nullptr; e->tsr_scratch_cap = 0;
    PT_HIP_CHECK(hipMalloc(&e->tsr_scratch, off));
    e->tsr_scratch_cap = off;
  }
  char* base = reinterpret_cast<char*>(e->tsr_scratch);
  float* sig = reinterpret_cast<float*>(base + o_sig);
  int* cnt = reinterpret_cast<int*>(base + o_cnt);
  auto* keys = reinterpret_cast<unsigned long long*>(base + o_keys);
  ds->cnt = cnt;
  ds->sorted = reinterpret_cast<unsigned long long*>(base + o_sorted);
  ds->boxes = reinterpret_cast<float*>(base + o_boxes);
  ds->rev = wiz_rev ? reinterpret_cast<float*>(base + o_rev) : nullptr;
  ds->keys2 = reinterpret_cast<unsigned long long*>(base + o_keys2);
  ds->sorted2 = wiz_rev ? reinterpret_cast<unsigned long long*>(base + o_sorted2) : nullptr;
  ds->sp_base = reinterpret_cast<int*>(base + o_sp);
  ds->sp_lim = ds->sp_base + B;
  ds->pk_base = ds->sp_lim + 2;
  ds->pk_lim = ds->pk_base + 2 * B;
  ds->wiz_rev = wiz_rev;
  PT_HIP_CHECK(hipMemsetAsync(cnt, 0, (size_t)B * 5 * 4, s));
  PT_HIP_CHECK(hipMemsetAsync(d_counts, 0, (size_t)B * 4, s));
  return pt_heat_peaks_topk(hm, B, H, W, vis_thresh, 0.3f, K_CELLS, K_CORNERS, sig, keys, cnt, ds->sorted, cnt + 2 * B, s);
}

static int decode_boxes(const DecodeState* ds, const float* reg0, const float* reg1, const float* wh, const float* st,
                        bool sparse, int B, int H, int W, hipStream_t s) {
  int* cnt = ds->cnt;
  hipLaunchKernelGGL(lore_boxes_kernel, dim3((K_CORNERS + 255) / 256, 2 * B), dim3(256), 0, s, ds->sorted, cnt + 2 * B, CAP, B,
                     H, W, reg0, reg1, wh, st, sparse ? (const int*)ds->pk_base : (const int*)nullptr, ds->boxes);
  if (ds->wiz_rev) {
    hipLaunchKernelGGL(lore_snap_kernel, dim3(K_CELLS, B), dim3(64), 0, s, ds->boxes, cnt + 2 * B, CAP, ds->rev);
    hipLaunchKernelGGL(lore_rekey_kernel, dim3((K_CELLS + 255) / 256, B), dim3(256), 0, s, ds->rev, cnt + 2 * B, CAP, ds->keys2);
    hipLaunchKernelGGL(lore_sort_kernel, dim3(B), dim3(1024), CAP * 8, s, ds->keys2, cnt + 2 * B, 2, CAP, K_CELLS, K_CELLS,
                       ds->sorted2, CAP, cnt + 4 * B, (const float*)nullptr, 0, 0, 0.f, 0.f);
  }
  PT_HIP_CHECK(hipGetLastError());
  return PT_OK;
}

int pt_lore_decode(pt_engine* e, const float* hm, const float* st, const float* wh, const float* ax, const float* cr,
                   const float* reg, int B, int H, int W, int wiz_rev, float vis_thresh, int* d_counts, float* d_dets,
                   float* d_logi, hipStream_t s) {
  PT_REQUIRE(hm && st && wh && ax && cr && reg && d_counts && d_dets && d_logi && B > 0, "tsr decode: null pointer");
  PtProfScope ps(e, s, PT_PROF_OTHER, 0, "tsr decode");
  DecodeState ds;
  int rc = decode_peaks(e, hm, B, H, W, wiz_rev, vis_thresh, d_counts, &ds, s);
  if (rc == PT_OK) rc = decode_boxes(&ds, reg, reg, wh, st, false, B, H, W, s);
  if (rc != PT_OK) return rc;
  hipLaunchKernelGGL(lore_gather_kernel, dim3(K_CELLS, B), dim3(256), 0, s, ds.rev, ds.boxes, ds.sorted2, ds.cnt + 2 * B, CAP, H,
                     W, ax, cr, vis_thresh, d_dets, d_logi, d_counts, (const int*)nullptr);
  PT_HIP_CHECK(hipGetLastError());
  return PT_OK;
}

void pt_lore_mosaic_rows(int B, int* rows_ax, int* rows_cr, int* rows_cell, int* rows_corner) {
  *rows_ax = (int)(((long long)B * K_CELLS + MOS_PW - 1) / MOS_PW);
  *rows_cr = (int)(((long long)B * K_CELLS * 4 + MOS_PW - 1) / MOS_PW);
  *rows_cell = *rows_ax;
  *rows_corner = (int)(((long long)B * K_CORNERS + MOS_PW - 1) / MOS_PW);
}

static_assert(sizeof(DecodeState) <= sizeof(pt_engine::tsr_decode_state), "DecodeState outgrew its slot in pt_engine");
#define g_ds (*reinterpret_cast<DecodeState*>(e->tsr_decode_state))

int pt_lore_decode_peaks(pt_engine* e, const float* hm, int B, int H, int W, int wiz_rev, float vis_thresh, int* d_counts,
                         const int** d_lim_cell, const int** d_lim_corner, hipStream_t s) {
  PT_REQUIRE(hm && d_counts && B > 0, "tsr decode peaks: null pointer");
  PtProfScope ps(e, s, PT_PROF_OTHER, 0, "tsr decode");
  int rc = decode_peaks(e, hm, B, H, W, wiz_rev, vis_thresh, d_counts, &g_ds, s);
  if (rc != PT_OK) return rc;
  hipLaunchKernelGGL(lore_peak_base_kernel, dim3(1), dim3(1), 0, s, g_ds.cnt + 2 * B, B, g_ds.pk_base, g_ds.pk_lim);
  PT_HIP_CHECK(hipGetLastError());
  *d_lim_cell = g_ds.pk_lim;
  *d_lim_corner = g_ds.pk_lim + 1;
  return PT_OK;
}

int pt_lore_peak_patches(pt_engine* e, const bf16_t* feat, int B, int H, int W, int C, int split, bf16_t* mos_cell,
                         bf16_t* mos_corner, hipStream_t s) {
  PT_REQUIRE(feat && mos_cell && mos_corner && C % 8 == 0, "tsr peak patches: bad arguments");
  PtProfScope ps(e, s, PT_PROF_OTHER, 0, "tsr patch gather");
  hipLaunchKernelGGL(lore_peak_patch_kernel, dim3(K_CORNERS, 2 * B), dim3(64), 0, s, g_ds.sorted, g_ds.cnt + 2 * B, CAP, H, W, feat,
                     C, split, g_ds.pk_base, mos_cell, mos_corner);
  PT_HIP_CHECK(hipGetLastError());
  return PT_OK;
}

int pt_lore_decode_boxes(pt_engine* e, const float* reg_cell, const float* wh, const float* reg_corner, const float* st, int B,
                         int H, int W, const int** d_lim_ax, const int** d_lim_cr, hipStream_t s) {
  PT_REQUIRE(reg_cell && wh && reg_corner && st, "tsr decode boxes: null pointer");
  PtProfScope ps(e, s, PT_PROF_OTHER, 0, "tsr decode");
  int rc = decode_boxes(&g_ds, reg_cell, reg_corner, wh, st, true, B, H, W, s);
  if (rc != PT_OK) return rc;
  hipLaunchKernelGGL(lore_sparse_base_kernel, dim3(1), dim3(1), 0, s, g_ds.cnt + 2 * B, B, g_ds.sp_base, g_ds.sp_lim);
  PT_HIP_CHECK(hipGetLastError());
  *d_lim_ax = g_ds.sp_lim;
  *d_lim_cr = g_ds.sp_lim + 1;
  return PT_OK;
}

int pt_lore_patch_gather(pt_engine* e, const bf16_t* feat, int B, int H, int W, int C, int split, bf16_t* mos_ax, bf16_t* mos_cr,
                         hipStream_t s) {
  PT_REQUIRE(feat && mos_ax && mos_cr && C % 8 == 0, "tsr patch gather: bad arguments");
  PtProfScope ps(e, s, PT_PROF_OTHER, 0, "tsr patch gather");
  hipLaunchKernelGGL(lore_patch_gather_kernel, dim3(K_CELLS, B), dim3(256), 0, s, g_ds.rev, g_ds.boxes, g_ds.sorted2,
                     g_ds.cnt + 2 * B, CAP, H, W, feat, C, split, g_ds.sp_base, mos_ax, mos_cr);
  PT_HIP_CHECK(hipGetLastError());
  return PT_OK;
}

int pt_lore_decode_sparse(pt_engine* e, const float* ax_mos, const float* cr_mos, int B, int H, int W, float vis_thresh,
                          int* d_counts, float* d_dets, float* d_logi, hipStream_t s) {
  PT_REQUIRE(ax_mos && cr_mos && d_counts && d_dets && d_logi, "tsr decode sparse: null pointer");
  PtProfScope ps(e, s, PT_PROF_OTHER, 0, "tsr decode");
  hipLaunchKernelGGL(lore_gather_kernel, dim3(K_CELLS, B), dim3(256), 0, s, g_ds.rev, g_ds.boxes, g_ds.sorted2, g_ds.cnt + 2 * B,
                     CAP, H, W, ax_mos, cr_mos, vis_thresh, d_dets, d_logi, d_counts, (const int*)g_ds.sp_base);
  PT_HIP_CHECK(hipGetLastError());
  return PT_OK;
}

}
```

pdf_table_amd/csrc/lore_model.hip:

```cpp
#include "dla_net.h"

namespace PT_FMT_NS {

int pt_launch_dcn_im2col(const bf16_t* x, const float* om, bf16_t* cols, int B, int H, int W, int C, int split,
                         hipStream_t s);
namespace {

struct Ctx : DlaCtx {
  struct UpTail {
    T p;
    const PtTensor* w = nullptr;
    int f = 0;
  };
  T dcn(const std::string& q, const T& x, int cout, const UpTail* up = nullptr) {
    T o = alloc(x.H, x.W, cout);
    static const bool fused = !(getenv("PT_DCN_FUSED") && atoi(getenv("PT_DCN_FUSED")) == 0);
    const bool om_inside = fused && pt_dcn_fuses_om(e, x.C, x3);
    if (!om_inside) conv(x, q + ".om", 64, 3, 1, T(), 0, nullptr, 32, om, 32, 0, 27);
    if (fused) {
      const PtTensor* w = get(q + (x3 ? ".dcn.w3" : ".dcn.w"));
      const PtTensor* b = get(q + ".dcn.b");
      const PtTensor* ow = om_inside ? get(q + (x3 ? ".om.w3" : ".om.w")) : nullptr;
      const PtTensor* ob = om_inside ? get(q + ".om.b") : nullptr;
      if (go()) {
// ... 20 lines not shown
    bool have_p = false, have_u = false;
    if (first_sum) { u = *first_sum; have_p = have_u = true; }
    for (int i = startp + 1; i < endp; ++i) {
      const int j = i - startp;
      const std::string js = std::to_string(j);
      if (!have_p) p = dcn(q + ".proj_" + js, layers[i], o_ch);
      if (!have_u) {
        const int f = up_f[j];
        u = alloc(p.H * f, p.W * f, o_ch);
        const PtTensor* wu = get(q + ".up_" + js + ".wf32");
        if (go()) {
          e->prof.next_bytes = (double)n * p.H * p.W * o_ch * 2.0 * mul * (1.0 + 2.0 * f * f);
          char label[48];
          snprintf(label, sizeof(label), "dw convT up + add %d @%dx%d", o_ch, p.H * f, p.W * f);
          PtProfScope ps(e, s, PT_PROF_OTHER, 0, label);
          const int r = pt_launch_dwconvt_up_add(p.p, F(wu), layers[i - 1].p, u.p, n, p.H, p.W, o_ch, f, x3, s);
          if (r != PT_OK) rc = r;
        }
      }
      have_p = have_u = false;
      UpTail nx;
      if (fuse && i + 1 < endp) {
        const std::string ns = std::to_string(j + 1);
        p = nx.p = dcn(q + ".proj_" + ns, layers[i + 1], o_ch);
        nx.w = get(q + ".up_" + ns + ".wf32");
        nx.f = up_f[j + 1];
        have_p = true;
      } else if (fuse && tail) {
        nx = *tail;
      }
      layers[i] = dcn(q + ".node_" + js, u, o_ch, nx.f ? &nx : nullptr);
      if (nx.f) { u = layers[i]; have_u = true; }
    }
  }
};

}

struct SparseArgs {
  int wiz_rev;
  float vis_thresh;
  int* d_counts;
  float *d_dets, *d_logi;
};

static int lore_dla_run(pt_engine* e, const bf16_t* x, int n, int H, int W, float* hm, float* st, float* wh, float* ax,
                        float* cr, float* reg, const SparseArgs* sp, hipStream_t s) {
  PT_REQUIRE(H % 32 == 0 && W % 32 == 0 && H > 0 && W > 0, "Lore net: input %dx%d must be multiples of 32", H, W);
  PT_REQUIRE(x && n > 0 && (sp || (hm && st && wh && ax && cr && reg)), "Lore net: null pointer");
  const PtModel* m = pt_find_model(e, PT_MODEL_LORE_DLA34, "Lore DLA-34", "PT_MODEL_LORE_DLA34");
  if (!m) return PT_ERR_STATE;
  Ctx c;
  c.init(e, m, "Lore DLA-34", s, n, PT_ARENA_TSR);
  float* heads[6] = {hm, st, wh, ax, cr, reg};
  const char* hname[6] = {"hm", "st", "wh", "ax", "cr", "reg"};
  const int hcs[6] = {8, 8, 8, 256, 256, 8};
  const int hreal[6] = {2, 8, 8, 256, 256, 2};

  return pt_plan_then_launch(c, "Lore net", [&]() -> int {
    const size_t px4 = (size_t)n * (H / 4) * (W / 4);
    c.cols = c.take<bf16_t>(px4 * 576 * c.mul * sizeof(bf16_t));
    c.om = c.take<float>(px4 * 32 * sizeof(float));

    std::vector<T> layers = dla34_base(c, x, H, W);

    std::vector<T> out = {layers[5]};
    const int f2[4] = {1, 2, 2, 2};
    c.ida("dla_up.ida_0", layers, 4, 6, 256, f2);
    out.insert(out.begin(), layers[5]);
    c.ida("dla_up.ida_1", layers, 3, 6, 128, f2);
    out.insert(out.begin(), layers[5]);
    const int f24[3] = {1, 2, 4};
    Ctx::UpTail t2;
    if (pt_dcn_fuses_up(e, 64, 64, c.x3)) {
      t2.p = c.dcn("ida_up.proj_1", out[0], 64);
      t2.w = c.get("ida_up.up_1.wf32");
      t2.f = f24[1];
    }
    c.ida("dla_up.ida_2", layers, 2, 6, 64, f2, true, t2.f ? &t2 : nullptr);
    out.insert(out.begin(), layers[5]);
    std::vector<T> y = {out[0], out[1], out[2]};
    c.ida("ida_up", y, 0, 3, 64, f24, true, nullptr, t2.f ? &y[0] : nullptr);
    const T feat = y[2];
    T hid = c.alloc(feat.H, feat.W, 256);
    if (sp) heads[0] = c.take<float>((size_t)n * feat.H * feat.W * 8 * sizeof(float));
    for (int h = 0; h < 6; ++h) {
      if (sp && h != 0) continue;
      c.conv(feat, std::string(hname[h]) + ".0", 256, 3, 1, hid, 1);
      c.conv(hid, std::string(hname[h]) + ".2", hcs[h] < 64 ? 64 : hcs[h], 1, 1, T(), 0, nullptr, hcs[h], heads[h], hcs[h], 0, hreal[h]);
    }
    if (sp) {
      int rows_ax = 0, rows_cr = 0, rows_cell = 0, rows_corner = 0;
      pt_lore_mosaic_rows(n, &rows_ax, &rows_cr, &rows_cell, &rows_corner);
      const int MW = 32;
      auto mosaic = [&](int rows, int C) {
        T t;
        t.H = rows; t.W = MW; t.C = C;
        t.p = c.take<bf16_t>(((size_t)rows * MW * C * c.mul + 64) * sizeof(bf16_t));
        return t;
      };
      T mcell = mosaic(rows_cell, 9 * 64), mcorner = mosaic(rows_corner, 9 * 64), max_ = mosaic(rows_ax, 9 * 64), mcr_ = mosaic(rows_cr, 9 * 64);
      T mhid = mosaic(rows_cr, 256);
      float* o_wh = c.take<float>((size_t)rows_cell * MW * 8 * sizeof(float));
      float* o_regc = c.take<float>((size_t)rows_cell * MW * 8 * sizeof(float));
      float* o_st = c.take<float>((size_t)rows_corner * MW * 8 * sizeof(float));
      float* o_regk = c.take<float>((size_t)rows_corner * MW * 8 * sizeof(float));
      float* oax = c.take<float>((size_t)rows_ax * MW * 256 * sizeof(float));
      float* ocr = c.take<float>((size_t)rows_cr * MW * 256 * sizeof(float));
      if (c.go()) {
        const int keep = c.n;
        auto head = [&](const T& mos, int rows, const char* name, int nc, float* outp, const int* lim, int real_nc) {
          T hh = mhid;
          hh.H = rows;
          c.n = 1;
          c.ylimit = lim;
          c.conv(mos, std::string(name) + ".0", 256, 1, 1, hh, 1);
          c.conv(hh, std::string(name) + ".2", nc < 64 ? 64 : nc, 1, 1, T(), 0, nullptr, nc, outp, nc, 0, real_nc);
          c.ylimit = nullptr;
          c.n = keep;
        };
        const int *lim_cell = nullptr, *lim_corner = nullptr, *lim_ax = nullptr, *lim_cr = nullptr;
        int r = pt_lore_decode_peaks(e, heads[0], n, feat.H, feat.W, sp->wiz_rev, sp->vis_thresh, sp->d_counts, &lim_cell,
                                     &lim_corner, s);
        if (r == PT_OK) r = pt_lore_peak_patches(e, feat.p, n, feat.H, feat.W, 64, c.x3, mcell.p, mcorner.p, s);
        if (r != PT_OK) return r;
        head(mcell, rows_cell, "wh", 8, o_wh, lim_cell, 8);
        head(mcell, rows_cell, "reg", 8, o_regc, lim_cell, 2);
        head(mcorner, rows_corner, "st", 8, o_st, lim_corner, 8);
        head(mcorner, rows_corner, "reg", 8, o_regk, lim_corner, 2);
        if (c.rc != PT_OK) return c.rc;
        r = pt_lore_decode_boxes(e, o_regc, o_wh, o_regk, o_st, n, feat.H, feat.W, &lim_ax, &lim_cr, s);
        if (r == PT_OK) r = pt_lore_patch_gather(e, feat.p, n, feat.H, feat.W, 64, c.x3, max_.p, mcr_.p, s);
        if (r != PT_OK) return r;
        head(max_, rows_ax, "ax", 256, oax, lim_ax, 256);
        head(mcr_, rows_cr, "cr", 256, ocr, lim_cr, 256);
        if (c.rc != PT_OK) return c.rc;
        r = pt_lore_decode_sparse(e, oax, ocr, n, feat.H, feat.W, sp->vis_thresh, sp->d_counts, sp->d_dets, sp->d_logi, s);
        if (r != PT_OK) return r;
      }
    }
    return c.rc;
  });
}


int pt_lore_forward_net(pt_engine* e, const bf16_t* x, int n, int H, int W, float* hm, float* st, float* wh, float* ax,
                        float* cr, float* reg, hipStream_t s) {
  PT_REQUIRE(hm && st && wh && ax && cr && reg, "Lore net: null pointer");
  return lore_dla_run(e, x, n, H, W, hm, st, wh, ax, cr, reg, nullptr, s);
}

int pt_lore_forward_decode(pt_engine* e, const bf16_t* x, int n, int H, int W, int wiz_rev, float vis_thresh, int* d_counts,
                           float* d_dets, float* d_logi, hipStream_t s) {
  PT_REQUIRE(d_counts && d_dets && d_logi, "Lore forward+decode: null pointer");
  SparseArgs sp{wiz_rev, vis_thresh, d_counts, d_dets, d_logi};
  return lore_dla_run(e, x, n, H, W, nullptr, nullptr, nullptr, nullptr, nullptr, nullptr, &sp, s);
}

namespace {

struct WCtx : NetCtx {
  void conv(const T& in, const std::string& q, int N, int ks, int stride, const T& out, int relu, const T* res = nullptr,
            int shuffle = 0, int nv = 0, float* out_f32 = nullptr, int f32_cs = 0) {
    ConvDesc c;
    if (!conv_desc(c, in, q, N, ks, stride, relu)) return;
    c.n_valid = nv; c.shuffle_cout = shuffle;
    if (shuffle && ks == 3) c.alg_scale = 16.0 / 36.0;
    if (out_f32) to_f32(c, out_f32, f32_cs);
    else to_map(c, out);
    if (res) { c.res = res->p; c.res_mode = 1; }
// ... 80 lines not shown
```

pdf_table_amd/engine.py:

```python
from __future__ import annotations

import contextlib
import ctypes as C
import functools
import threading
from typing import Optional, Sequence, Tuple

import numpy as np
import torch

from . import lib as L

__all__ = ["HipEngine", "REC_LINE_DTYPE", "CLS_IMAGE_DTYPE", "REC_PP_ITEM_DTYPE"]

TSR_TABLE_DTYPE = np.dtype([("minv", "<f8", (6,)), ("page", "<i4"), ("x0", "<i4"), ("y0", "<i4"),
                            ("crop_w", "<i4"), ("crop_h", "<i4"), ("reserved", "<i4")])
CLS_IMAGE_DTYPE = np.dtype([("offset", "<i8"), ("h", "<i4"), ("w", "<i4")])
REC_LINE_DTYPE = np.dtype([("minv", np.float64, (9,)), ("page", np.int32), ("crop_w", np.int32), ("crop_h", np.int32),
                           ("reserved", np.int32)])


REC_PP_ITEM_DTYPE = np.dtype([("line", "<i4"), ("resized_w", "<i4"), ("img_w", "<i4"), ("reserved", "<i4"),
                              ("out_off", "<i8")])

# ... 593 lines not shown

    def op_conv2d(self, x: torch.Tensor, w_tiled: torch.Tensor, bias: torch.Tensor, ks: int, stride: int = 1,
                  relu: bool = False, res: Optional[torch.Tensor] = None, res_mode: int = 0, rep: int = 1,
                  shuffle_cout: int = 0, out: Optional[torch.Tensor] = None, out_coff: int = 0,
                  split: int = 0) -> torch.Tensor:
        self._chk(x, self.act_dtype, "x")
        self._chk(bias, torch.float32, "bias")
        B, H, W, Cin = x.shape
        m = 2 if split else 1
        Cin //= m
        N = bias.numel()
        pad = ks // 2
        Ho, Wo = (H + 2 * pad - ks) // stride + 1, (W + 2 * pad - ks) // stride + 1
        if out is None:
            if shuffle_cout:
                out = torch.empty((B, 2 * Ho, 2 * Wo, shuffle_cout * m), dtype=self.act_dtype, device=self._tdev)
            else:
                out = torch.empty((B, Ho * rep, Wo * rep, N * m), dtype=self.act_dtype, device=self._tdev)
        L.check(self.lib.pt_op_conv2d(self._h, _ptr(x), B, H, W, Cin, _ptr(w_tiled), _ptr(bias), N, ks, stride,
                                      _ptr(out), out.shape[-1], out_coff, rep, shuffle_cout, _ptr(res), res_mode,
                                      int(relu), int(split), out.shape[-1] // 2, self._stream()), "pt_op_conv2d")
        return out

    def op_conv1x1_ex(self, x: torch.Tensor, w_tiled: torch.Tensor, bias: torch.Tensor, relu: int = 0, out_f32: bool = False,
                      n_valid: int = 0, res_f32: Optional[torch.Tensor] = None, ylimit: Optional[torch.Tensor] = None) -> torch.Tensor:
        self._chk(x, self.act_dtype, "x")
        self._chk(bias, torch.float32, "bias")
        B, H, W, Cin = x.shape
        N = bias.numel()
        cs = n_valid or N
        out = torch.zeros((B, H, W, cs), dtype=torch.float32 if out_f32 else self.act_dtype, device=self._tdev)
        L.check(self.lib.pt_op_conv1x1_ex(self._h, _ptr(x), B, H, W, Cin, _ptr(w_tiled), _ptr(bias), N, None if out_f32 else _ptr(out),
                                          _ptr(out) if out_f32 else None, cs, n_valid, _ptr(res_f32), int(relu), _ptr(ylimit),
                                          self._stream()), "pt_op_conv1x1_ex")
        return out

    def op_dcn(self, x: torch.Tensor, om: torch.Tensor, w_tiled: torch.Tensor, bias: torch.Tensor, relu: bool = True, split: int = 0) -> torch.Tensor:
        self._chk(x, self.act_dtype, "x")
        self._chk(om, torch.float32, "om")
        self._chk(bias, torch.float32, "bias")
        B, H, W, Cc = x.shape
        m = 2 if split else 1
        Cc //= m
        if tuple(om.shape) != (B, H, W, 32):
            raise ValueError(f"op_dcn: om must be [B,H,W,32], got {tuple(om.shape)}")
        N = bias.numel()
        out = torch.empty((B, H, W, N * m), dtype=self.act_dtype, device=self._tdev)
        L.check(self.lib.pt_op_dcn(self._h, _ptr(x), _ptr(om), B, H, W, Cc, _ptr(w_tiled), _ptr(bias), N, _ptr(out), int(relu), int(split),
                                   self._stream()), "pt_op_dcn")
        return out

    def op_dwconvt_up_add(self, x: torch.Tensor, w_taps: torch.Tensor, add: Optional[torch.Tensor], f: int, split: int = 0) -> torch.Tensor:
        self._chk(x, self.act_dtype, "x")
        self._chk(w_taps, torch.float32, "w_taps")
        B, h, w, Cc = x.shape
        if add is not None:
            self._chk(add, self.act_dtype, "add")
            if tuple(add.shape) != (B, h * f, w * f, Cc):
                raise ValueError(f"op_dwconvt_up_add: add must be {(B, h * f, w * f, Cc)}, got {tuple(add.shape)}")
        out = torch.empty((B, h * f, w * f, Cc), dtype=self.act_dtype, device=self._tdev)
        L.check(self.lib.pt_op_dwconvt_up_add(self._h, _ptr(x), _ptr(w_taps), _ptr(add), _ptr(out), B, h, w, Cc // 2 if split else Cc, int(f),
                                              int(split), self._stream()), "pt_op_dwconvt_up_add")
        return out

    def op_dcn_up_add(self, x: torch.Tensor, om: torch.Tensor, w_tiled: torch.Tensor, bias: torch.Tensor, up_in: torch.Tensor, up_taps: torch.Tensor,
                      f: int, relu: bool = True, split: int = 0) -> torch.Tensor:
        self._chk(x, self.act_dtype, "x")
        self._chk(om, torch.float32, "om")
        self._chk(bias, torch.float32, "bias")
        self._chk(up_in, self.act_dtype, "up_in")
        self._chk(up_taps, torch.float32, "up_taps")
        B, H, W, Cc = x.shape
        if tuple(om.shape) != (B, H, W, 32):
            raise ValueError(f"op_dcn_up_add: om must be [B,H,W,32], got {tuple(om.shape)}")
        N = bias.numel()
        if up_in.dim() != 4 or up_in.shape[0] != B or up_in.shape[3] != N:
            raise ValueError(f"op_dcn_up_add: up_in must be [{B},h,w,{N}], got {tuple(up_in.shape)}")
        out = torch.empty((B, H, W, N), dtype=self.act_dtype, device=self._tdev)
        L.check(self.lib.pt_op_dcn_up_add(self._h, _ptr(x), _ptr(om), B, H, W, Cc // 2 if split else Cc, _ptr(w_tiled), _ptr(bias), N, _ptr(out), int(relu),
                                          int(split), _ptr(up_in), up_in.shape[1], up_in.shape[2], _ptr(up_taps), int(f), self._stream()),
                "pt_op_dcn_up_add")
        return out

    def op_dwconv(self, x: torch.Tensor, w_taps: torch.Tensor, bias: torch.Tensor, k: int, stride: int = 1, act: int = 0, split: bool = False) -> torch.Tensor:
        self._chk(x, self.act_dtype, "x")
        self._chk(w_taps, torch.float32, "w_taps")
        self._chk(bias, torch.float32, "bias")
        B, H, W, Cc = x.shape
        pad = k // 2
        out = torch.empty((B, (H + 2 * pad - k) // stride + 1, (W + 2 * pad - k) // stride + 1, Cc), dtype=self.act_dtype, device=self._tdev)
        L.check(self.lib.pt_op_dwconv(self._h, _ptr(x), B, H, W, Cc // 2 if split else Cc, _ptr(w_taps), _ptr(bias), k, stride, act, _ptr(out), int(split),
                                      self._stream()), "pt_op_dwconv")
        return out

    def op_add(self, a: torch.Tensor, b: torch.Tensor, split: bool = False) -> torch.Tensor:
        self._chk(a, self.act_dtype, "a")
        self._chk(b, self.act_dtype, "b")
        if a.shape != b.shape:
            raise ValueError(f"op_add: shapes differ: {tuple(a.shape)} vs {tuple(b.shape)}")
        out = torch.empty_like(a)
        L.check(self.lib.pt_op_add(self._h, _ptr(a), _ptr(b), _ptr(out), a.numel() // a.shape[-1], a.shape[-1] // 2 if split else a.shape[-1], int(split),
                                   self._stream()), "pt_op_add")
        return out

    def op_maxpool(self, x: torch.Tensor, k: int, stride: int, pad: int, split: bool = False) -> torch.Tensor:
        self._chk(x, self.act_dtype, "x")
        B, H, W, Cc = x.shape
        out = torch.empty((B, (H + 2 * pad - k) // stride + 1, (W + 2 * pad - k) // stride + 1, Cc), dtype=self.act_dtype, device=self._tdev)
        L.check(self.lib.pt_op_maxpool(self._h, _ptr(x), B, H, W, Cc // 2 if split else Cc, k, stride, pad, _ptr(out), int(split), self._stream()), "pt_op_maxpool")
        return out

    def op_avgpool(self, x: torch.Tensor, k: int, split: bool = False) -> torch.Tensor:
        self._chk(x, self.act_dtype, "x")
        B, H, W, Cc = x.shape
        out = torch.empty((B, H // k, W // k, Cc), dtype=self.act_dtype, device=self._tdev)
        L.check(self.lib.pt_op_avgpool(self._h, _ptr(x), B, H, W, Cc // 2 if split else Cc, k, _ptr(out), int(split), self._stream()), "pt_op_avgpool")
        return out

    def op_conv2d_rect(self, x: torch.Tensor, w_tiled: torch.Tensor, bias: torch.Tensor, kh: int, kw: int, sh: int = 1, sw: int = 1, act: int = 0,
                       out: Optional[torch.Tensor] = None, out_coff: int = 0, split: int = 0) -> torch.Tensor:
        self._chk(x, self.act_dtype, "x")
        self._chk(bias, torch.float32, "bias")
        B, H, W, Cin = x.shape
        m = 2 if split else 1
        Cin //= m
        N = bias.numel()
        Ho, Wo = (H + 2 * (kh // 2) - kh) // sh + 1, (W + 2 * (kw // 2) - kw) // sw + 1
        if out is None:
            out = torch.empty((B, Ho, Wo, N * m), dtype=self.act_dtype, device=self._tdev)
        else:
            self._chk(out, self.act_dtype, "out")
            if tuple(out.shape[:3]) != (B, Ho, Wo):
                raise ValueError(f"op_conv2d_rect: out must be [{B},{Ho},{Wo},C], got {tuple(out.shape)}")
        L.check(self.lib.pt_op_conv2d_rect(self._h, _ptr(x), B, H, W, Cin, _ptr(w_tiled), _ptr(bias), N, kh, kw, sh, sw, _ptr(out), out.shape[-1],
                                           out_coff, int(act), int(split), out.shape[-1] // 2, self._stream()), "pt_op_conv2d_rect")
        return out

    def op_conv2d_large(self, x: torch.Tensor, w_tiled: torch.Tensor, bias: torch.Tensor, kh: int, kw: int, act: int = 0,
                        out: Optional[torch.Tensor] = None, out_coff: int = 0, split: int = 0) -> torch.Tensor:
        self._chk(x, self.act_dtype, "x")
        self._chk(bias, torch.float32, "bias")
        B, H, W, Cin = x.shape
        m = 2 if split else 1
        Cin //= m
        N = bias.numel()
        if out is None:
            out = torch.empty((B, H, W, N * m), dtype=self.act_dtype, device=self._tdev)
        else:
            self._chk(out, self.act_dtype, "out")
            if tuple(out.shape[:3]) != (B, H, W):
                raise ValueError(f"op_conv2d_large: out must be [{B},{H},{W},C], got {tuple(out.shape)}")
        L.check(self.lib.pt_op_conv2d_large(self._h, _ptr(x), B, H, W, Cin, _ptr(w_tiled), _ptr(bias), N, kh, kw, _ptr(out), out.shape[-1],
                                            out_coff, int(act), int(split), out.shape[-1] // 2, self._stream()), "pt_op_conv2d_large")
        return out

    def op_dwconv_rect(self, x: torch.Tensor, w_taps: torch.Tensor, bias: torch.Tensor, k: int, sh: int, sw: int, act: int = 0, split: bool = False) -> torch.Tensor:
        self._chk(x, self.act_dtype, "x")
        self._chk(w_taps, torch.float32, "w_taps")
        self._chk(bias, torch.float32, "bias")
        B, H, W, Cc = x.shape
        pad = k // 2
        out = torch.empty((B, (H + 2 * pad - k) // max(sh, 1) + 1, (W + 2 * pad - k) // max(sw, 1) + 1, Cc), dtype=self.act_dtype, device=self._tdev)
        L.check(self.lib.pt_op_dwconv_rect(self._h, _ptr(x), B, H, W, Cc // 2 if split else Cc, _ptr(w_taps), _ptr(bias), k, sh, sw, act, _ptr(out),
                                           int(split), self._stream()), "pt_op_dwconv_rect")
        return out

# ... 328 lines not shown
```

pdf_table_amd/lib.py:

```python
from __future__ import annotations

import ctypes as C
import os

_HERE = os.path.dirname(os.path.abspath(__file__))
LIB_PATH = os.environ.get("PT_LIB_PATH") or os.path.join(_HERE, "libpdftable_hip.so")

PT_MODEL_DB_RESNET18 = 1
PT_MODEL_CRNN = 2
PT_MODEL_LORE_DLA34 = 3
PT_MODEL_LORE_PROCESSOR = 4
PT_MODEL_PICODET = 5
PT_MODEL_LORE_RESNET18 = 6
PT_MODEL_DB_NAS = 7
PT_MODEL_PPLCNET = 8
PT_MODEL_CONVNEXT_VIT = 16
PT_MODEL_MTL_BACKBONE = 17
PT_MODEL_MTL_DECODER = 18
PT_MODEL_CENTERNET_DLA34 = 19
PT_CVIT_W, PT_CVIT_CHUNK_W, PT_CVIT_CHUNK_STEP, PT_CVIT_T, PT_CVIT_NCLS = 804, 300, 252, 201, 7644
PT_CLS_SLOTS = 4
PT_CLS_MAX_CLASSES = 16
PT_LAYOUT_HEAD_CS, PT_LAYOUT_CAND_FLOATS = 40, 48
PT_DET_PRE_DB_PP = 0
# ... 9 lines not shown
PT_CENTERNET_MAX_CELLS = 1000
PT_ROTATE_90_CLOCKWISE, PT_ROTATE_180, PT_ROTATE_90_COUNTERCLOCKWISE = 0, 1, 2
PT_REC_H, PT_REC_W, PT_REC_T, PT_REC_NCLS = 32, 640, 160, 7644
PT_PROF_CLASSES = ("conv3x3", "conv1x1", "stem", "other")
EXPECTED_ABI = 19

_lib = None


class PtError(RuntimeError):
    pass


def _proto(lib):
    vp, i, f, sz = C.c_void_p, C.c_int, C.c_float, C.c_size_t
    ip = C.POINTER(C.c_int)
    P = {
        "pt_engine_create": (i, [i, C.POINTER(vp)]),
        "pt_engine_destroy": (None, [vp]),
        "pt_last_error": (C.c_char_p, []),
        "pt_abi_version": (i, []),
        "pt_engine_check": (i, [vp]),
        "pt_engine_set_precision": (i, [vp, i]),
        "pt_engine_set_lstm_cluster": (i, [vp, i]),
        "pt_engine_set_mtl_kv_fp8": (i, [vp, i]),
        "pt_engine_set_dcn_mfma": (i, [vp, i]),
        "pt_weights_load": (i, [vp, i, vp, sz]),
        "pt_weights_load_device": (i, [vp, i, vp, sz, vp]),
        "pt_det_plan": (i, [i, i, i, ip, ip]),
        "pt_det_forward": (i, [vp, vp, i, i, i, i, f, i, vp, vp, vp]),
        "pt_det_forward_net": (i, [vp, vp, i, i, i, vp, vp, vp]),
        "pt_det_preprocess": (i, [vp, vp, i, i, i, i, vp, vp]),
        "pt_det_bitmap": (i, [vp, vp, i, i, i, f, i, vp, vp]),
        "pt_det_box_scores": (i, [vp, vp, i, i, i, vp, i, vp, vp]),
        "pt_db_candidates": (i, [vp, i, i, i, f, vp, vp, i, ip]),
        "pt_db_finalize": (i, [vp, vp, i, f, f, f, i, i, i, i, i, vp, vp, i, ip]),
        "pt_db_candidates_batch": (i, [vp, i, i, i, i, f, i, vp, vp, i, vp]),
        "pt_db_finalize_batch": (i, [vp, vp, vp, i, i, f, f, f, i, i, i, i, i, i, i, vp, vp, vp, vp]),
        "pt_rec_forward": (i, [vp, vp, i, i, i, vp, vp, i, vp, vp, vp]),
        "pt_rec_forward_crops": (i, [vp, vp, vp, vp, i, vp, vp, vp]),
        "pt_rec_forward_net": (i, [vp, vp, i, vp, vp, vp]),
        "pt_rec_preprocess": (i, [vp, vp, i, i, i, vp, vp, i, vp, vp]),
        "pt_rec_cvit_forward": (i, [vp, vp, i, i, i, vp, vp, vp, i, vp, vp, vp]),
        "pt_rec_cvit_forward_crops": (i, [vp, vp, vp, vp, vp, i, vp, vp, vp]),
        "pt_rec_cvit_forward_net": (i, [vp, vp, i, i, vp, vp, vp, vp]),
        "pt_rec_cvit_preprocess_crops": (i, [vp, vp, vp, vp, i, vp, vp]),
        "pt_tsr_mtl_backbone_net": (i, [vp, vp, i, i, i, vp, vp]),
        "pt_tsr_mtl_preprocess": (i, [vp, vp, i, i, i, vp, i, i, vp, vp]),
        "pt_tsr_mtl_resized_size": (None, [i, i, i, ip, ip]),
        "pt_tsr_mtl_decoder_config": (i, [vp, ip]),
        "pt_tsr_mtl_structure": (i, [vp, vp, i, i, vp, vp, ip, ip, i, vp]),
        "pt_tsr_mtl_cells": (i, [vp, i, vp, vp, vp, ip, i, vp]),
        "pt_rec_pp_preprocess": (i, [vp, vp, i, i, i, vp, vp, i, vp, i, i, i, vp, vp]),
        "pt_rec_pp_preprocess_crops": (i, [vp, vp, vp, vp, i, vp, i, i, i, vp, vp]),
        "pt_layout_plan": (i, [i, i, ip, ip]),
        "pt_layout_preprocess": (i, [vp, vp, i, i, i, i, i, vp, vp]),
        "pt_layout_forward_net": (i, [vp, vp, i, i, i, vp, vp, vp, vp, vp]),
        "pt_layout_candidates": (i, [vp, vp, vp, vp, vp, i, i, i, i, f, i, vp, vp, vp]),
        "pt_layout_forward": (i, [vp, vp, i, i, i, i, i, i, f, i, vp, vp, vp]),
        "pt_tsr_preprocess": (i, [vp, vp, i, i, i, vp, i, i, i, i, vp, vp]),
        "pt_tsr_forward_net": (i, [vp, vp, i, i, i, vp, vp, vp, vp, vp, vp, vp]),
        "pt_tsr_forward_net_wireless": (i, [vp, vp, i, i, i, vp, vp, vp, vp, vp, vp, vp]),
        "pt_tsr_decode": (i, [vp, vp, vp, vp, vp, vp, vp, i, i, i, i, f, vp, vp, vp, vp]),
        "pt_tsr_forward_decode": (i, [vp, vp, i, i, i, i, f, vp, vp, vp, vp]),
        "pt_tsr_process": (i, [vp, vp, vp, vp, i, i, vp, vp, vp]),
        "pt_centernet_forward_net": (i, [vp, vp, i, i, i, vp, vp, vp, vp, vp]),
        "pt_centernet_decode": (i, [vp, vp, vp, vp, vp, i, i, i, vp, vp, vp, vp]),
        "pt_hard_nms": (i, [vp, vp, vp, i, C.c_double, i, vp, vp]),
        "pt_page_line_mask": (i, [vp, i, i, i, vp, vp]),
        "pt_page_line_angles": (i, [vp, i, i, i, i, i, vp, i, vp]),
        "pt_page_warp_cubic": (i, [vp, i, i, i, vp, vp, i, vp, vp]),
        "pt_page_quarter_turn": (i, [vp, i, i, i, i, vp, vp]),
        "pt_page_pre_tables": (i, [vp, vp]),
        "pt_cls_preprocess": (i, [vp, vp, vp, i, i, i, i, i, vp, vp]),
        "pt_cls_forward_net": (i, [vp, i, vp, i, i, i, i, vp, ip, vp]),
        "pt_cls_forward": (i, [vp, i, vp, vp, i, i, i, i, i, i, vp, ip, vp]),
        "pt_cls_forward_lines": (i, [vp, i, vp, i, i, i, vp, vp, i, i, i, i, i, i, vp, ip, vp]),
        "pt_cls_forward_lines_direct": (i, [vp, i, vp, i, i, i, vp, i, i, i, i, i, i, vp, ip, vp]),
        "pt_op_conv2d": (i, [vp, vp, i, i, i, i, vp, vp, i, i, i, vp, i, i, i, i, vp, i, i, i, i, vp]),
        "pt_op_conv1x1_ex": (i, [vp, vp, i, i, i, i, vp, vp, i, vp, vp, i, i, vp, i, vp, vp]),
        "pt_op_dcn": (i, [vp, vp, vp, i, i, i, i, vp, vp, i, vp, i, i, vp]),
        "pt_op_dwconvt_up_add": (i, [vp, vp, vp, vp, vp, i, i, i, i, i, i, vp]),
        "pt_op_dcn_up_add": (i, [vp, vp, vp, i, i, i, i, vp, vp, i, vp, i, i, vp, i, i, vp, i, vp]),
        "pt_op_stem7x7": (i, [vp, vp, i, i, i, vp, vp, vp, i, vp]),
        "pt_op_maxpool3x3s2": (i, [vp, vp, i, i, i, i, vp, i, vp]),
        "pt_op_db_head_final": (i, [vp, vp, i, i, i, vp, vp, vp, vp, i, vp]),
        "pt_op_dwconv": (i, [vp, vp, i, i, i, i, vp, vp, i, i, i, vp, i, vp]),
        "pt_op_add": (i, [vp, vp, vp, vp, C.c_longlong, i, i, vp]),
        "pt_op_maxpool": (i, [vp, vp, i, i, i, i, i, i, i, vp, i, vp]),
        "pt_op_avgpool": (i, [vp, vp, i, i, i, i, i, vp, i, vp]),
        "pt_op_chan_mean": (i, [vp, vp, i, i, i, vp, vp, i, vp]),
        "pt_op_chan_mean_scratch_floats": (i, [i, i]),
        "pt_op_scale_channels": (i, [vp, vp, vp, i, i, i, vp, i, vp]),
        "pt_op_act": (i, [vp, vp, C.c_longlong, i, C.c_float, C.c_float, vp, i, i, vp]),
        "pt_op_copy_channels": (i, [vp, vp, C.c_longlong, i, i, vp, i, i, i, vp]),
        "pt_op_upsample_nearest": (i, [vp, vp, i, i, i, i, i, vp, vp]),
        "pt_op_mul": (i, [vp, vp, vp, vp, C.c_longlong, i, i, vp]),
        "pt_copy_bytes": (i, [vp, vp, vp, C.c_longlong, vp]),
        "pt_op_layernorm": (i, [vp, vp, C.c_longlong, i, i, vp, vp, C.c_float, vp, i, vp]),
        "pt_op_softmax": (i, [vp, vp, C.c_longlong, i, i, vp, vp, i, vp]),
        "pt_op_attention": (i, [vp, vp, i, i, i, i, i, C.c_float, vp, i, i, vp]),
        "pt_op_lstm": (i, [vp, vp, i, vp, i, i, i, i, i, vp, i, i, vp]),
        "pt_op_lstm_packed_elems": (i, [i, i, i]),
        "pt_op_cvit_mlp": (i, [vp, vp, C.c_longlong, i, vp, vp, vp, vp, vp, vp]),
        "pt_op_cvit_attention": (i, [vp, vp, i, vp, i, vp]),
        "pt_op_cvit_dwconv_ln": (i, [vp, vp, i, i, i, i, vp, vp, vp, vp, vp, i, vp]),
        "pt_op_cvit_ln": (i, [vp, vp, C.c_longlong, i, vp, vp, C.c_float, vp, i, i, i, i, vp, vp]),
        "pt_op_conv2d_rect": (i, [vp, vp, i, i, i, i, vp, vp, i, i, i, i, i, vp, i, i, i, i, i, vp]),
        "pt_op_conv2d_large": (i, [vp, vp, i, i, i, i, vp, vp, i, i, i, vp, i, i, i, i, i, vp]),
        "pt_op_dwconv_rect": (i, [vp, vp, i, i, i, i, vp, vp, i, i, i, i, vp, i, vp]),
        "pt_op_pool_rect": (i, [vp, vp, i, i, i, i, i, i, i, vp, i, vp]),
        "pt_op_affine_act": (i, [vp, vp, C.c_longlong, i, i, vp, vp, vp, vp, i, vp, i, vp]),
        "pt_op_db_tail": (i, [vp, vp, i, i, i, i, i, i, vp, vp, vp, vp, vp, i, vp]),
        "pt_profile_enable": (i, [vp, i]),
        "pt_profile_read": (i, [vp, vp, vp, vp]),
        "pt_profile_read_labels": (i, [vp, C.c_char_p, i]),
    }
    for name, (res, args) in P.items():
        try:
            fn = getattr(lib, name)
        except AttributeError:
            raise PtError(f"{LIB_PATH} does not export {name}: it was built from older sources; rebuild it (`python -m pdf_table_amd.build --force`)") from None
        fn.restype = res
        fn.argtypes = args
    return P


EXPORTS = None


def load():
    global _lib, EXPORTS
    if _lib is None:
        import torch
        if not os.path.exists(LIB_PATH):
            raise PtError(f"{LIB_PATH} not found: run `python -m pdf_table_amd.build` (hipcc, gfx950). "
                          "There is no CPU fallback.")
        lib = C.CDLL(LIB_PATH, mode=C.RTLD_GLOBAL)
        EXPORTS = _proto(lib)
        have = int(lib.pt_abi_version())
        if have != EXPECTED_ABI:
            raise PtError(f"{LIB_PATH} reports ABI {have}, this binding was written for ABI {EXPECTED_ABI}: rebuild it "
                          "(`python -m pdf_table_amd.build --force`)")
        _lib = lib
    return _lib


def check(rc: int, what: str = ""):
    if rc != 0:
        msg = load().pt_last_error()
        raise PtError(f"{what} failed (status {rc}): {msg.decode() if msg else '?'}")
```

Measured before the change: 791.9.

## Fuse LORE heat-map 1x1 head and sigmoid into the persistent 3x3 conv epilogue

Adds a heat-map variant of the persistent 3x3 pipelined conv kernel. In its epilogue it applies bias and ReLU, reduces the 256 hidden channels against the two-class 1x1 weights using a register carry plus an LDS exchange across the two N-tiles, and writes either the logits or the sigmoid scores straight into the decode scratch buffer. This avoids writing and re-reading the 256-channel hidden map, a second GEMM launch, and in the decode path a separate sigmoid kernel. The cost is extra LDS, a block barrier per tile pair, and tiles assigned to blocks in pairs, which can worsen load balance. It is on by default when the DMA, variant-3 pipe conv path is active.

```diff
diff --git a/include/pdftable_hip.h b/include/pdftable_hip.h
--- a/include/pdftable_hip.h
+++ b/include/pdftable_hip.h
@@ -206,6 +206,10 @@
 int pt_op_dcn_up_add(pt_engine* e, const uint16_t* d_in, const float* d_om, int B, int H, int W, int C, const uint16_t* d_w_tiled,
                      const float* d_bias, int N, uint16_t* d_out, int relu, int split, const uint16_t* d_up_in, int up_h, int up_w,
                      const float* d_up_w, int up_f, pt_stream stream);
+
+int pt_op_lore_hm_head(pt_engine* e, const uint16_t* d_in, int B, int H, int W, const uint16_t* d_w1_tiled, const float* d_b1,
+                       const uint16_t* d_w2_tiled, const float* d_b2, int fused, uint16_t* d_hid, float* d_logits, float* d_sig, float* d_sig_ref,
+                       pt_stream stream);
 
 int pt_op_stem7x7(pt_engine* e, const uint16_t* d_in, int B, int H, int W, const uint16_t* d_w, const float* d_bias,
                   uint16_t* d_out, int split, pt_stream stream);
diff --git a/pdf_table_amd/csrc/c_api.hip b/pdf_table_amd/csrc/c_api.hip
--- a/pdf_table_amd/csrc/c_api.hip
+++ b/pdf_table_amd/csrc/c_api.hip
@@ -1000,6 +1000,34 @@
                              d_up_in, d_up_w, up_f);
 }
 
+int pt_op_lore_hm_head(pt_engine* e, const uint16_t* d_in, int B, int H, int W, const uint16_t* d_w1_tiled, const float* d_b1, const uint16_t* d_w2_tiled,
+                       const float* d_b2, int fused, uint16_t* d_hid, float* d_logits, float* d_sig, float* d_sig_ref, pt_stream stream) {
+  PT_REQUIRE(e && d_in && d_w1_tiled && d_b1 && d_w2_tiled && d_b2, "pt_op_lore_hm_head: null argument");
+  PT_REQUIRE(B > 0 && H > 0 && W > 0, "pt_op_lore_hm_head: empty map (B=%d H=%d W=%d)", B, H, W);
+  PT_REQUIRE(!pt_split(e), "pt_op_lore_hm_head: single-pass modes only");
+  PT_REQUIRE(d_logits || (fused && d_sig), "pt_op_lore_hm_head: no output");
+  PT_REQUIRE(!d_sig_ref || d_logits, "pt_op_lore_hm_head: d_sig_ref is computed from d_logits");
+  hipStream_t s = reinterpret_cast<hipStream_t>(stream);
+  ConvDesc d;
+  d.in = d_in; d.B = B; d.H = H; d.W = W; d.Cin = 64; d.w = d_w1_tiled; d.bias = d_b1; d.N = 256; d.ks = 3; d.stride = 1; d.relu = 1;
+  int rc;
+  if (fused) {
+    PT_REQUIRE(pt_conv_fuses_hm(e), "pt_op_lore_hm_head: the fused head is switched off (PT_LORE_HM_FUSE / PT_CONV_PIPE / PT_CONV_DMA / PT_CONV_VARIANT)");
+    d.hm_w2 = d_w2_tiled; d.hm_b2 = d_b2; d.hm_logits = d_logits; d.hm_sig = d_sig;
+    if ((rc = pt_launch_conv(e, d, s)) != PT_OK) return rc;
+  } else {
+    PT_REQUIRE(d_hid && d_logits && !d_sig, "pt_op_lore_hm_head: the two launches write d_hid and d_logits (scores: d_sig_ref)");
+    d.out = d_hid; d.out_cstride = 256;
+    if ((rc = pt_launch_conv(e, d, s)) != PT_OK) return rc;
+    ConvDesc d2;
+    d2.in = d_hid; d2.B = B; d2.H = H; d2.W = W; d2.Cin = 256; d2.w = d_w2_tiled; d2.bias = d_b2; d2.N = 64; d2.ks = 1; d2.stride = 1;
+    d2.n_valid = 8; d2.out_f32 = d_logits; d2.out_cstride = 8; d2.alg_n = 2;
+    if ((rc = pt_launch_conv(e, d2, s)) != PT_OK) return rc;
+  }
+  if (d_sig_ref) return pt_launch_heat_sigmoid(d_logits, d_sig_ref, (long long)B * H * W, s);
+  return PT_OK;
+}
+
 int pt_profile_enable(pt_engine* e, int on) {
   PT_REQUIRE(e != nullptr, "pt_profile_enable: null engine");
   PT_REQUIRE(on >= 0 && on < 2 + PT_PROF_NCLASS, "pt_profile_enable: mode %d out of range", on);
diff --git a/pdf_table_amd/csrc/common.h b/pdf_table_amd/csrc/common.h
--- a/pdf_table_amd/csrc/common.h
+++ b/pdf_table_amd/csrc/common.h
@@ -244,8 +244,13 @@
   int xp_store = 0;
   int alg_n = 0;
   double alg_scale = 1.0;
+  const bf16_t* hm_w2 = nullptr;
+  const float* hm_b2 = nullptr;
+  float* hm_logits = nullptr;
+  float* hm_sig = nullptr;
 };
 int pt_launch_conv(pt_engine* e, const ConvDesc& d, hipStream_t s);
+bool pt_conv_fuses_hm(const pt_engine* e);
 int pt_launch_crnn_conv01(pt_engine* e, const bf16_t* gray, int n, const float* w64x9, const float* b0, const bf16_t* w1, const float* b1, bf16_t* p1,
                           const int* xlimit, const int* xlimit_cols, hipStream_t s);
 int pt_launch_dwpw(pt_engine* e, const bf16_t* in, int B, int H, int W, int C, const float* dw_w, const float* dw_b, int k, int stride, int dw_act,
@@ -376,6 +381,9 @@
                     int use_2dpe, float* d_logic, float* d_stacked, hipStream_t s);
 int pt_lore_forward_net(pt_engine* e, const bf16_t* x, int n, int H, int W, float* hm, float* st, float* wh, float* ax,
                         float* cr, float* reg, hipStream_t s);
+__device__ __forceinline__ float pt_heat_sigmoid(float x) { return 1.f / (1.f + expf(-x)); }
+int pt_launch_heat_sigmoid(const float* hm, float* sig, long long npix, hipStream_t s);
+int pt_lore_decode_sig_map(pt_engine* e, int B, int H, int W, float** d_sig);
 constexpr int PT_HEAT_CAP = 16384;
 int pt_heat_peaks_topk(const float* hm, int B, int H, int W, float thr0, float thr1, int k0, int k1, float* sig, unsigned long long* keys,
                        int* cnt, unsigned long long* sorted, int* kept, hipStream_t s);
diff --git a/pdf_table_amd/csrc/conv_igemm.hip b/pdf_table_amd/csrc/conv_igemm.hip
--- a/pdf_table_amd/csrc/conv_igemm.hip
+++ b/pdf_table_amd/csrc/conv_igemm.hip
@@ -1336,11 +1336,21 @@
 }
 
 template <int NT, int NWV, int S>
-__global__ __launch_bounds__(64 * NWV, 2) void conv3x3_pipe_persist_kernel(ConvK p) {
+struct PersistHm {
+  using C = PipeCfg<NT, NWV, 0, S>;
+  static constexpr int PAR_FLOATS = 3 * 256 + 8;
+  static constexpr int PAR_BYTES = (PAR_FLOATS * 4 + 255) & ~255;
+  static constexpr int XCH_BYTES = (NWV / 2) * C::MT * 64 * 4;
+  static constexpr int SMEM = 2 * C::BUF_BYTES + PAR_BYTES + XCH_BYTES;
+  static_assert(SMEM <= 163840, "LDS budget");
+};
+
 #if defined(__HIP_DEVICE_COMPILE__)
-  a16_kernel_enter();
+template <int NT, int NWV, int S, bool HM>
+__device__ __forceinline__ void conv3x3_pipe_persist_body(const ConvK& p) {
   using C = PipeCfg<NT, NWV, 0, S>;
   static_assert(C::NBLK == 1, "ordinary tiles");
+  static_assert(!HM || (NT == 2 && S == 1), "fused head: the 128-channel stride-1 tile");
   extern __shared__ __attribute__((aligned(16))) char smem[];
   const int tid = threadIdx.x;
   const int lane = tid & 63;
@@ -1350,8 +1360,24 @@
   const int wn = NT == 1 ? 0 : (wave & 1);
   const int G = gridDim.x;
   const int Lw = xcd_remap(blockIdx.x, G);
-  const int t0 = (int)((long long)Lw * p.total_tiles / G), t1 = (int)((long long)(Lw + 1) * p.total_tiles / G);
+  const int cut = HM ? 2 : 1, units = p.total_tiles / cut;
+  const int t0 = cut * (int)((long long)Lw * units / G), t1 = cut * (int)((long long)(Lw + 1) * units / G);
   if (t0 >= t1) return;
+  float* const hm_par = reinterpret_cast<float*>(smem + 2 * C::BUF_BYTES);
+  float* const hm_xch = reinterpret_cast<float*>(smem + 2 * C::BUF_BYTES + PersistHm<NT, NWV, S>::PAR_BYTES);
+  float hm_carry[C::MT];
+  if constexpr (HM) {
+    const bf16_t* hm_w2 = static_cast<const bf16_t*>(p.head_w);
+    if (tid < 256) {
+      hm_par[tid] = p.bias[tid];
+      hm_par[256 + tid] = bf16_to_f32(hm_w2[((tid >> 5) * 64 + 0) * 32 + (tid & 31)]);
+      hm_par[512 + tid] = bf16_to_f32(hm_w2[((tid >> 5) * 64 + 1) * 32 + (tid & 31)]);
+    } else if (tid < 264) {
+      hm_par[768 + tid - 256] = p.head_b[tid - 256];
+    }
+#pragma unroll
+    for (int m = 0; m < C::MT; ++m) hm_carry[m] = 0.f;
+  }
   const int in_cs = p.Cin;
   const int nch32 = p.Cin >> 5, nslices = nch32 * 2;
 
@@ -1499,7 +1525,72 @@
       r_w = rsrc_w(cur);
     }
     skew_slice(nslices - 1, std::integral_constant<int, 1>{}, std::true_type{}, 0, 0);
-    {
+    if constexpr (HM) {
+      const int n0 = (done.nb * 2 + wn) * 64;
+      float part[C::MT][2];
+#pragma unroll
+      for (int m = 0; m < C::MT; ++m) part[m][0] = part[m][1] = 0.f;
+#pragma unroll
+      for (int nb = 0; nb < 2; ++nb)
+#pragma unroll
+        for (int g = 0; g < 4; ++g) {
+          const int ch = n0 + nb * 32 + 8 * g + 4 * qh;
+          const f32x4 bv = *reinterpret_cast<const f32x4*>(hm_par + ch);
+          const f32x4 w0 = *reinterpret_cast<const f32x4*>(hm_par + 256 + ch);
+          const f32x4 w1 = *reinterpret_cast<const f32x4*>(hm_par + 512 + ch);
+#pragma unroll
+          for (int m = 0; m < C::MT; ++m) {
+            const uint32_t d0 = pack_bf16x2(fmaxf(acc[m][nb][4 * g + 0] + bv.x, 0.f), fmaxf(acc[m][nb][4 * g + 1] + bv.y, 0.f));
+            const uint32_t d1 = pack_bf16x2(fmaxf(acc[m][nb][4 * g + 2] + bv.z, 0.f), fmaxf(acc[m][nb][4 * g + 3] + bv.w, 0.f));
+            const float h0 = bf16lo_f32(d0), h1 = bf16hi_f32(d0), h2 = bf16lo_f32(d1), h3 = bf16hi_f32(d1);
+            part[m][0] = fmaf(h0, w0.x, part[m][0]); part[m][1] = fmaf(h0, w1.x, part[m][1]);
+            part[m][0] = fmaf(h1, w0.y, part[m][0]); part[m][1] = fmaf(h1, w1.y, part[m][1]);
+            part[m][0] = fmaf(h2, w0.z, part[m][0]); part[m][1] = fmaf(h2, w1.z, part[m][1]);
+            part[m][0] = fmaf(h3, w0.w, part[m][0]); part[m][1] = fmaf(h3, w1.w, part[m][1]);
+          }
+        }
+#pragma unroll
+      for (int m = 0; m < C::MT; ++m)
+#pragma unroll
+        for (int n = 0; n < 2; ++n)
+#pragma unroll
+          for (int r = 0; r < 16; ++r) acc[m][n][r] = 0.f;
+      float cur[C::MT];
+#pragma unroll
+      for (int m = 0; m < C::MT; ++m) {
+        const u32x2 sw = __builtin_amdgcn_permlane32_swap(__float_as_uint(part[m][0]), __float_as_uint(part[m][1]), false, false);
+        cur[m] = __uint_as_float(sw.x) + __uint_as_float(sw.y);
+      }
+      if (done.nb == 0) {
+#pragma unroll
+        for (int m = 0; m < C::MT; ++m) hm_carry[m] = cur[m];
+      } else {
+#pragma unroll
+        for (int m = 0; m < C::MT; ++m) {
+          cur[m] = hm_carry[m] + cur[m];
+          if (wn == 1) hm_xch[(wm * C::MT + m) * 64 + lane] = cur[m];
+        }
+        __syncthreads();
+        if (wn == 0) {
+          const float b2 = hm_par[768 + qh];
+#pragma unroll
+          for (int m = 0; m < C::MT; ++m) {
+            const float lg = (cur[m] + hm_xch[(wm * C::MT + m) * 64 + lane]) + b2;
+            const int oy = done.oy0 + C::MT * wm + m, ox = done.ox0 + lx;
+            const bool inside = oy < p.Ho && ox < p.Wo;
+            const size_t pix = ((size_t)done.b * p.Ho + oy) * p.Wo + ox;
+            if (p.head_prob && inside) p.head_prob[2 * pix + qh] = pt_heat_sigmoid(lg);
+            if (p.head_logits) {
+              const u32x2 sw = __builtin_amdgcn_permlane32_swap(__float_as_uint(lg), __float_as_uint(lg), false, false);
+              const f32x4 pad = *reinterpret_cast<const f32x4*>(hm_par + 768 + 4 * qh);
+              f32x4 o = {0.f + pad.x, 0.f + pad.y, 0.f + pad.z, 0.f + pad.w};
+              if (qh == 0) { o.x = __uint_as_float(sw.x); o.y = __uint_as_float(sw.y); }
+              if (inside) *reinterpret_cast<f32x4*>(p.head_logits + 8 * pix + 4 * qh) = o;
+            }
+          }
+        }
+      }
+    } else {
       const int n0 = (NT == 1 ? done.nb : done.nb * 2 + wn) * 64;
       const DirectBias bs = direct_bias<2>(p, n0, qh);
 #pragma unroll
@@ -1513,6 +1604,22 @@
     }
     load_frags(smem, 0, 0);
   }
+}
+#endif
+
+template <int NT, int NWV, int S>
+__global__ __launch_bounds__(64 * NWV, 2) void conv3x3_pipe_persist_kernel(ConvK p) {
+#if defined(__HIP_DEVICE_COMPILE__)
+  a16_kernel_enter();
+  conv3x3_pipe_persist_body<NT, NWV, S, false>(p);
+#endif
+}
+
+template <int NT, int NWV, int S>
+__global__ __launch_bounds__(64 * NWV, 2) void conv3x3_pipe_persist_hm_kernel(ConvK p) {
+#if defined(__HIP_DEVICE_COMPILE__)
+  a16_kernel_enter();
+  conv3x3_pipe_persist_body<NT, NWV, S, true>(p);
 #endif
 }
 
@@ -2995,6 +3102,36 @@
   return PT_OK;
 }
 
+static int launch_pipe_persist_hm(pt_engine* e, ConvK& k, hipStream_t s, double flop) {
+  using C = PipeCfg<2, 8, 0, 1>;
+  using HM = PersistHm<2, 8, 1>;
+  static bool attr_done = false;
+  if (!attr_done) {
+    PT_HIP_CHECK(hipFuncSetAttribute(reinterpret_cast<const void*>(&conv3x3_pipe_persist_hm_kernel<2, 8, 1>), hipFuncAttributeMaxDynamicSharedMemorySize, HM::SMEM));
+    attr_done = true;
+  }
+  k.n_tiles = k.N / C::NW;
+  k.tiles_x = (k.Wo + C::TW - 1) / C::TW;
+  k.tiles_y = (k.Ho + C::TH - 1) / C::TH;
+  const long long ptiles = (long long)k.B * k.tiles_x * k.tiles_y, total = ptiles * k.n_tiles;
+  PT_REQUIRE(k.n_tiles == 2 && total > 0 && total < (1ll << 31), "conv grid out of range (%lld tiles)", total);
+  k.total_tiles = (int)total;
+  long long grid = e->num_cu;
+  if (const char* gv = getenv("PT_CONV_PERSIST_GRID")) {
+    const int gg = atoi(gv);
+    if (gg > 0) grid = gg;
+  }
+  if (grid > ptiles) grid = ptiles;
+  char label[48];
+  snprintf(label, sizeof(label), "conv3x3 v5+hm %d->%d->2 @%dx%d", k.Cin, k.N, k.Ho, k.Wo);
+  {
+    PtProfScope prof(e, s, PT_PROF_CONV3X3, flop, label);
+    hipLaunchKernelGGL((conv3x3_pipe_persist_hm_kernel<2, 8, 1>), dim3((unsigned)grid), dim3(C::NTHR), HM::SMEM, s, k);
+  }
+  PT_HIP_CHECK(hipGetLastError());
+  return PT_OK;
+}
+
 static int launch_gemm_pipe(pt_engine* e, ConvK& k, hipStream_t s, double flop) {
   using C = GemmPipeCfg;
   static bool attr_done = false;
@@ -3071,8 +3208,14 @@
   return v;
 }
 
+bool pt_conv_fuses_hm(const pt_engine* e) {
+  const char* ev = getenv("PT_LORE_HM_FUSE");
+  const char* pv = getenv("PT_CONV_PIPE");
+  return !pt_split(e) && use_dma_kernel() && conv_variant() == 3 && !(pv && atoi(pv) < 4) && !(ev && atoi(ev) == 0);
+}
+
 int pt_launch_conv(pt_engine* e, const ConvDesc& d, hipStream_t s) {
-  PT_REQUIRE(d.in && d.w && d.bias && (d.out || d.out_f32 || d.head_w || d.argmax_part), "conv: null pointer");
+  PT_REQUIRE(d.in && d.w && d.bias && (d.out || d.out_f32 || d.head_w || d.argmax_part || d.hm_w2), "conv: null pointer");
   PT_REQUIRE(d.Cin % 32 == 0 && d.Cin > 0, "conv: Cin=%d must be a positive multiple of 32", d.Cin);
   PT_REQUIRE(d.N % 64 == 0 && d.N > 0, "conv: N=%d must be a positive multiple of 64", d.N);
   PT_REQUIRE((d.ks == 1 || d.ks == 3) && (d.stride == 1 || d.stride == 2), "conv: ks=%d stride=%d unsupported", d.ks,
@@ -3135,6 +3278,17 @@
     if (d.res || d.res_f32) by += (double)k.B * k.Ho * k.Wo * nstore * (d.res_f32 ? 4.0 : 2.0 * mact) / (d.res_mode == 2 ? 4.0 : 1.0);
     by += (double)d.N * d.Cin * d.ks * d.ks * 2.0 * (d.split == 2 ? 2 : (d.split ? 3 : 1));
     e->prof.next_bytes = by;
+  }
+  if (d.hm_w2) {
+    PT_REQUIRE(pt_conv_fuses_hm(e) && d.ks == 3 && d.stride == 1 && d.Cin == 64 && d.N == 256 && d.relu == 1 && !d.res && !d.res_f32 && !d.split && d.nseg <= 1 &&
+                   !d.n_valid && !d.out_f32 && !d.head_w && !d.argmax_part && !d.ylimit && !d.xlimit && !d.xlimit_rows && !d.pool && d.rep == 1 && !d.shuffle_cout,
+               "conv: the fused heat-map head is the plain 3x3 64 -> 256 + ReLU layer in a single-pass mode");
+    PT_REQUIRE(d.hm_b2 && (d.hm_logits || d.hm_sig), "conv: fused heat-map head without bias or output");
+    for (int i = 0; i < 8; ++i) PT_REQUIRE(d.tap_mask[i] == 0, "conv: fused heat-map head with a tap mask");
+    k.head_w = d.hm_w2; k.head_b = d.hm_b2; k.head_logits = d.hm_logits; k.head_prob = d.hm_sig;
+    const double px = (double)k.B * k.Ho * k.Wo;
+    e->prof.next_bytes = px * d.Cin * 2.0 + px * ((d.hm_logits ? 8 : 0) + (d.hm_sig ? 2 : 0)) * 4.0 + (double)d.N * d.Cin * 9 * 2.0 + 2.0 * d.N * 2.0;
+    return launch_pipe_persist_hm(e, k, s, flop + 2.0 * px * d.N * 2.0);
   }
   if (d.ks == 3 && d.stride == 2 && !d.split && d.N % 128 == 0 && d.Cin % 32 == 0 && d.Cin >= 64 && k.Ho >= 8 && !d.head_w && !d.argmax_part && !d.n_valid &&
       !d.out_f32 && !d.res_f32 && !d.res && d.relu < 2 && !d.ylimit && !d.xlimit && !d.xlimit_rows && !d.pool && d.rep == 1 && !d.shuffle_cout && use_dma_kernel()) {
diff --git a/pdf_table_amd/csrc/lore_decode.hip b/pdf_table_amd/csrc/lore_decode.hip
--- a/pdf_table_amd/csrc/lore_decode.hip
+++ b/pdf_table_amd/csrc/lore_decode.hip
@@ -12,8 +12,8 @@
   a16_kernel_enter();
   const long long i = (long long)blockIdx.x * blockDim.x + threadIdx.x;
   if (i >= npix) return;
-  sig[2 * i] = 1.f / (1.f + expf(-hm[8 * i]));
-  sig[2 * i + 1] = 1.f / (1.f + expf(-hm[8 * i + 1]));
+  sig[2 * i] = pt_heat_sigmoid(hm[8 * i]);
+  sig[2 * i + 1] = pt_heat_sigmoid(hm[8 * i + 1]);
 }
 
 __device__ __forceinline__ bool heat_is_peak(const float* __restrict__ sb, int H, int W, int y, int x, int cls, float thr, float& s) {
@@ -441,7 +441,7 @@
 
 int pt_heat_peaks_topk(const float* hm, int B, int H, int W, float thr0, float thr1, int k0, int k1, float* sig, unsigned long long* keys,
                        int* cnt, unsigned long long* sorted, int* kept, hipStream_t s) {
-  PT_REQUIRE(hm && sig && keys && cnt && sorted && kept && B > 0 && k0 <= CAP && k1 <= CAP, "heat peaks: bad arguments");
+  PT_REQUIRE(sig && keys && cnt && sorted && kept && B > 0 && k0 <= CAP && k1 <= CAP, "heat peaks: bad arguments");
   PT_REQUIRE((long long)H * W < (1ll << 31), "heat peaks: map too large");
   static bool attr_done = false;
   if (!attr_done) {
@@ -450,10 +450,17 @@
     attr_done = true;
   }
   const size_t npix = (size_t)B * H * W;
-  hipLaunchKernelGGL(lore_sigmoid_kernel, dim3((unsigned)((npix + 255) / 256)), dim3(256), 0, s, hm, sig, (long long)npix);
+  if (hm) hipLaunchKernelGGL(lore_sigmoid_kernel, dim3((unsigned)((npix + 255) / 256)), dim3(256), 0, s, hm, sig, (long long)npix);
   hipLaunchKernelGGL(lore_peaks_kernel<1024>, dim3((unsigned)((npix + 1023) / 1024)), dim3(1024), 0, s, sig, B, H, W, thr0, thr1, keys, cnt);
   hipLaunchKernelGGL(lore_sort_kernel, dim3(2 * B), dim3(1024), CAP * 8, s, keys, cnt, 1, CAP, k0, k1, sorted, CAP, kept,
                      (const float*)sig, H, W, thr0, thr1);
+  PT_HIP_CHECK(hipGetLastError());
+  return PT_OK;
+}
+
+int pt_launch_heat_sigmoid(const float* hm, float* sig, long long npix, hipStream_t s) {
+  PT_REQUIRE(hm && sig && npix > 0, "heat sigmoid: bad arguments");
+  hipLaunchKernelGGL(lore_sigmoid_kernel, dim3((unsigned)((npix + 255) / 256)), dim3(256), 0, s, hm, sig, npix);
   PT_HIP_CHECK(hipGetLastError());
   return PT_OK;
 }
@@ -467,22 +474,50 @@
   int wiz_rev;
 };
 
+struct DecodeCarve {
+  size_t o_sig, o_cnt, o_keys, o_sorted, o_boxes, o_rev, o_keys2, o_sorted2, o_sp, total;
+};
+static DecodeCarve decode_carve(int B, int H, int W) {
+  const size_t npix = (size_t)B * H * W;
+  size_t off = 0;
+  auto carve = [&](size_t bytes) { size_t o = off; off = (off + bytes + 255) & ~size_t(255); return o; };
+  DecodeCarve c;
+  c.o_sig = carve(npix * 2 * 4); c.o_cnt = carve((size_t)B * 5 * 4); c.o_keys = carve((size_t)2 * B * CAP * 8);
+  c.o_sorted = carve((size_t)2 * B * CAP * 8); c.o_boxes = carve((size_t)2 * B * CAP * 12 * 4);
+  c.o_rev = carve((size_t)B * CAP * 12 * 4); c.o_keys2 = carve((size_t)B * CAP * 8);
+  c.o_sorted2 = carve((size_t)B * CAP * 8); c.o_sp = carve((size_t)(3 * B + 4) * 4);
+  c.total = off;
+  return c;
+}
+static int decode_scratch(pt_engine* e, const DecodeCarve& c) {
+  if (c.total > e->tsr_scratch_cap) {
+    PT_HIP_CHECK(hipDeviceSynchronize());
+    if (e->tsr_scratch) PT_HIP_CHECK(hipFree(e->tsr_scratch));
+    e->tsr_scratch = nullptr; e->tsr_scratch_cap = 0;
+    PT_HIP_CHECK(hipMalloc(&e->tsr_scratch, c.total));
+    e->tsr_scratch_cap = c.total;
+  }
+  return PT_OK;
+}
+
+int pt_lore_decode_sig_map(pt_engine* e, int B, int H, int W, float** d_sig) {
+  PT_REQUIRE(e && d_sig && B > 0 && H > 0 && W > 0, "tsr decode score map: bad arguments");
+  const DecodeCarve c = decode_carve(B, H, W);
+  const int rc = decode_scratch(e, c);
+  if (rc != PT_OK) return rc;
+  *d_sig = reinterpret_cast<float*>(reinterpret_cast<char*>(e->tsr_scratch) + c.o_sig);
+  return PT_OK;
+}
+
 static int decode_peaks(pt_engine* e, const float* hm, int B, int H, int W, int wiz_rev, float vis_thresh, int* d_counts,
                         DecodeState* ds, hipStream_t s) {
   PT_REQUIRE((long long)H * W < (1ll << 31), "tsr decode: map too large");
-  const size_t npix = (size_t)B * H * W;
-  size_t off = 0;
-  auto carve = [&](size_t bytes) { size_t o = off; off = (off + bytes + 255) & ~size_t(255); return o; };
-  const size_t o_sig = carve(npix * 2 * 4), o_cnt = carve((size_t)B * 5 * 4), o_keys = carve((size_t)2 * B * CAP * 8),
-               o_sorted = carve((size_t)2 * B * CAP * 8), o_boxes = carve((size_t)2 * B * CAP * 12 * 4),
-               o_rev = carve((size_t)B * CAP * 12 * 4), o_keys2 = carve((size_t)B * CAP * 8),
-               o_sorted2 = carve((size_t)B * CAP * 8), o_sp = carve((size_t)(3 * B + 4) * 4);
-  if (off > e->tsr_scratch_cap) {
-    PT_HIP_CHECK(hipDeviceSynchronize());
-    if (e->tsr_scratch) PT_HIP_CHECK(hipFree(e->tsr_scratch));
-    e->tsr_scratch = nullptr; e->tsr_scratch_cap = 0;
-    PT_HIP_CHECK(hipMalloc(&e->tsr_scratch, off));
-    e->tsr_scratch_cap = off;
+  const DecodeCarve c = decode_carve(B, H, W);
+  const size_t o_sig = c.o_sig, o_cnt = c.o_cnt, o_keys = c.o_keys, o_sorted = c.o_sorted, o_boxes = c.o_boxes, o_rev = c.o_rev, o_keys2 = c.o_keys2,
+               o_sorted2 = c.o_sorted2, o_sp = c.o_sp;
+  {
+    const int rc = decode_scratch(e, c);
+    if (rc != PT_OK) return rc;
   }
   char* base = reinterpret_cast<char*>(e->tsr_scratch);
   float* sig = reinterpret_cast<float*>(base + o_sig);
@@ -546,7 +581,7 @@
 
 int pt_lore_decode_peaks(pt_engine* e, const float* hm, int B, int H, int W, int wiz_rev, float vis_thresh, int* d_counts,
                          const int** d_lim_cell, const int** d_lim_corner, hipStream_t s) {
-  PT_REQUIRE(hm && d_counts && B > 0, "tsr decode peaks: null pointer");
+  PT_REQUIRE(d_counts && B > 0, "tsr decode peaks: null pointer");
   PtProfScope ps(e, s, PT_PROF_OTHER, 0, "tsr decode");
   int rc = decode_peaks(e, hm, B, H, W, wiz_rev, vis_thresh, d_counts, &g_ds, s);
   if (rc != PT_OK) return rc;
diff --git a/pdf_table_amd/csrc/lore_model.hip b/pdf_table_amd/csrc/lore_model.hip
--- a/pdf_table_amd/csrc/lore_model.hip
+++ b/pdf_table_amd/csrc/lore_model.hip
@@ -126,10 +126,27 @@
     std::vector<T> y = {out[0], out[1], out[2]};
     c.ida("ida_up", y, 0, 3, 64, f24, true, nullptr, t2.f ? &y[0] : nullptr);
     const T feat = y[2];
-    T hid = c.alloc(feat.H, feat.W, 256);
-    if (sp) heads[0] = c.take<float>((size_t)n * feat.H * feat.W * 8 * sizeof(float));
+    const bool hm_fused = pt_conv_fuses_hm(e);
+    T hid;
+    if (!(sp && hm_fused)) hid = c.alloc(feat.H, feat.W, 256);
+    if (sp && !hm_fused) heads[0] = c.take<float>((size_t)n * feat.H * feat.W * 8 * sizeof(float));
     for (int h = 0; h < 6; ++h) {
       if (sp && h != 0) continue;
+      if (h == 0 && hm_fused) {
+        const PtTensor* w2 = c.get("hm.2.w");
+        const PtTensor* b2 = c.get("hm.2.b");
+        ConvDesc d;
+        if (!c.conv_desc(d, feat, "hm.0", 256, 3, 1, 1)) continue;
+        d.hm_w2 = c.W(w2); d.hm_b2 = c.F(b2);
+        if (sp) {
+          const int r = pt_lore_decode_sig_map(e, n, feat.H, feat.W, &d.hm_sig);
+          if (r != PT_OK) return r;
+        } else {
+          d.hm_logits = heads[0];
+        }
+        c.launch(d);
+        continue;
+      }
       c.conv(feat, std::string(hname[h]) + ".0", 256, 3, 1, hid, 1);
       c.conv(hid, std::string(hname[h]) + ".2", hcs[h] < 64 ? 64 : hcs[h], 1, 1, T(), 0, nullptr, hcs[h], heads[h], hcs[h], 0, hreal[h]);
     }
diff --git a/pdf_table_amd/engine.py b/pdf_table_amd/engine.py
--- a/pdf_table_amd/engine.py
+++ b/pdf_table_amd/engine.py
@@ -699,6 +699,24 @@
                 "pt_op_dcn_up_add")
         return out
 
+    def op_lore_hm_head(self, feat: torch.Tensor, w1_tiled: torch.Tensor, b1: torch.Tensor, w2_tiled: torch.Tensor, b2: torch.Tensor,
+                        fused: bool, want_sig: bool = False, want_sig_ref: bool = False, logits_fill: float = 0.0):
+        self._chk(feat, self.act_dtype, "feat")
+        self._chk(b1, torch.float32, "b1")
+        self._chk(b2, torch.float32, "b2")
+        B, H, W, Cc = feat.shape
+        if Cc != 64 or b1.numel() != 256 or b2.numel() != 64:
+            raise ValueError(f"op_lore_hm_head: feat [B,H,W,64], b1 [256], b2 [64]; got {tuple(feat.shape)}, {b1.numel()}, {b2.numel()}")
+        if want_sig and not fused:
+            raise ValueError("op_lore_hm_head: the two launches have no score output of their own (want_sig_ref)")
+        logits = torch.full((B, H, W, 8), float(logits_fill), dtype=torch.float32, device=self._tdev)
+        hid = None if fused else torch.empty((B, H, W, 256), dtype=self.act_dtype, device=self._tdev)
+        sig = torch.zeros((B, H, W, 2), dtype=torch.float32, device=self._tdev) if want_sig else None
+        sig_ref = torch.zeros((B, H, W, 2), dtype=torch.float32, device=self._tdev) if want_sig_ref else None
+        L.check(self.lib.pt_op_lore_hm_head(self._h, _ptr(feat), B, H, W, _ptr(w1_tiled), _ptr(b1), _ptr(w2_tiled), _ptr(b2), int(bool(fused)), _ptr(hid),
+                                            _ptr(logits), _ptr(sig), _ptr(sig_ref), self._stream()), "pt_op_lore_hm_head")
+        return dict(logits=logits, hid=hid, sig=sig, sig_ref=sig_ref)
+
     def op_dwconv(self, x: torch.Tensor, w_taps: torch.Tensor, bias: torch.Tensor, k: int, stride: int = 1, act: int = 0, split: bool = False) -> torch.Tensor:
         self._chk(x, self.act_dtype, "x")
         self._chk(w_taps, torch.float32, "w_taps")
diff --git a/pdf_table_amd/lib.py b/pdf_table_amd/lib.py
--- a/pdf_table_amd/lib.py
+++ b/pdf_table_amd/lib.py
@@ -115,6 +115,7 @@
         "pt_op_dcn": (i, [vp, vp, vp, i, i, i, i, vp, vp, i, vp, i, i, vp]),
         "pt_op_dwconvt_up_add": (i, [vp, vp, vp, vp, vp, i, i, i, i, i, i, vp]),
         "pt_op_dcn_up_add": (i, [vp, vp, vp, i, i, i, i, vp, vp, i, vp, i, i, vp, i, i, vp, i, vp]),
+        "pt_op_lore_hm_head": (i, [vp, vp, i, i, i, vp, vp, vp, vp, i, vp, vp, vp, vp, vp]),
         "pt_op_stem7x7": (i, [vp, vp, i, i, i, vp, vp, vp, i, vp]),
         "pt_op_maxpool3x3s2": (i, [vp, vp, i, i, i, i, vp, i, vp]),
         "pt_op_db_head_final": (i, [vp, vp, i, i, i, vp, vp, vp, vp, i, vp]),
```

New measurement: 810.5, median of 6. 1.02x the previous value.
